# karpathy/minbpe

Measured on AMD Instinct MI355X. Metric: BPE merges/sec, higher is better.
Workload: dtype int32; 1 GPU; regex1g: RegexTokenizer.train, 1 GB synth seed 2, vocab 32000; mode=default, parallelism=single

## Files before the change

### minbpe_amd/_native.py

```python
import ctypes as C
import os
import sys

import numpy as np

_HERE = os.path.dirname(os.path.abspath(__file__))
LIB_PATH = os.environ.get("MINBPE_AMD_LIB", os.path.join(_HERE, "lib", "libbpe_hip.so"))

BPE_OK = 0
BPE_E_HIP = -1
BPE_E_ARG = -2
BPE_E_EMPTY_STATS = -3
BPE_E_STATE = -4
BPE_E_CAP = -5
BPE_E_LIMIT = -6
BPE_E_INTERNAL = -7

PROF_KINDS = ("widen", "pair_count", "argmax", "merge", "table", "encode", "decode")

if not os.path.exists(LIB_PATH):
    raise ImportError(
        f"{LIB_PATH} is missing: build it with `python -m minbpe_amd.build` "
        "(hipcc --offload-arch=gfx950). minbpe_amd has no CPU fallback.")

# ... 387 lines not shown
                return 1

        cb = ALLREDUCE_FN(_cb)
        rc = _lib.bpe_dp_train_cb(self._h, num_merges, rank, nranks, C.cast(cb, C.c_void_p), None, _ptr(pairs),
                                  _ptr(counts), _ptr(lens), C.byref(done))
        d = done.value
        self.last_train = dict(
            pairs=list(map(tuple, pairs[:2 * d].reshape(d, 2).tolist())),
            counts=counts[:d].tolist(), lens=lens[:d].tolist(), iter_ms=None, n_done=d)
        if raised:
            raise raised[0]
        self._check(rc)
        return self.last_train

    def encode_batch(self, pairs, merge_ids, data, offsets=None):
        buf = np.frombuffer(data, dtype=np.uint8) if not isinstance(data, np.ndarray) else data
        off, n_off = self._offsets(offsets)
        n_chunks = n_off if off is not None else 1
        pm = np.ascontiguousarray(pairs, dtype=np.int32).reshape(-1)
        M = len(pm) // 2
        mi = None if merge_ids is None else np.ascontiguousarray(merge_ids, dtype=np.int32)
        out = np.empty(max(len(buf), 1), np.int32)
        oo = np.zeros(n_chunks + 1, np.uint64)
        n_out = _u64(0)
        self._check(_lib.bpe_encode_batch(self._h, _ptr(pm) if M else None, _ptr(mi), M,
                                          _ptr(buf) if len(buf) else None, len(buf), _ptr(off),
                                          n_off, _ptr(out), _ptr(oo), C.byref(n_out)))
        return out[:n_out.value], oo

    def encode_batch_resident(self, pairs, merge_ids, d_bytes: int, n: int, d_offsets: int, n_chunks: int,
                              d_ids_out: int, d_out_offsets: int) -> int:
        p = np.ascontiguousarray(pairs, dtype=np.int32).reshape(-1)
        mids = None if merge_ids is None else np.ascontiguousarray(merge_ids, dtype=np.int32)
        total = _u64(0)
        self._check(_lib.bpe_encode_batch_resident(
            self._h, _ptr(p) if len(p) else None, None if mids is None else _ptr(mids), len(p) // 2,
            C.c_void_p(d_bytes), n, C.c_void_p(d_offsets), n_chunks, C.c_void_p(d_ids_out), C.c_void_p(d_out_offsets),
            C.byref(total)))
        return int(total.value)

    def decode_set_vocab(self, blob: bytes, offsets):
        buf = np.frombuffer(blob, dtype=np.uint8)
        off = np.ascontiguousarray(offsets, dtype=np.uint64)
        self._check(_lib.bpe_decode_set_vocab(self._h, _ptr(buf) if len(buf) else None, _ptr(off),
                                              len(off) - 1))

    def decode_batch(self, ids, doc_offsets=None):
        arr = np.ascontiguousarray(ids, dtype=np.int32)
        nb, bad = _u64(0), _u64(0)
        rc = _lib.bpe_decode_batch(self._h, _ptr(arr) if len(arr) else None, len(arr), C.byref(nb),
                                   C.byref(bad))
        if rc == BPE_E_ARG and bad.value != 0xFFFFFFFFFFFFFFFF:
            raise InvalidToken(int(bad.value))
        self._check(rc)
        out = np.empty(max(nb.value, 1), np.uint8)
        if doc_offsets is None:
            self._check(_lib.bpe_decode_read(self._h, _ptr(out), len(out), None, 0, None))
            return out[:nb.value].tobytes()
        doff = np.ascontiguousarray(doc_offsets, dtype=np.uint64)
        boff = np.zeros(len(doff), np.uint64)
        self._check(_lib.bpe_decode_read(self._h, _ptr(out), len(out), _ptr(doff), len(doff), _ptr(boff)))
        return out[:nb.value].tobytes(), boff

    def decode_set_sparse(self, sparse_ids, v_dense: int):
        arr = np.ascontiguousarray(sparse_ids, dtype=np.int32)
        self._check(_lib.bpe_decode_set_sparse(self._h, _ptr(arr) if len(arr) else None, len(arr), int(v_dense)))

    def decode_batch_resident(self, d_ids: int, id_width: int, n: int, d_doc_off: int, k: int, d_out: int, out_cap: int,
                              d_boff: int) -> int:
        nb, bad = _u64(0), _u64(0)
        rc = _lib.bpe_decode_batch_resident(self._h, C.c_void_p(d_ids), id_width, n, C.c_void_p(d_doc_off), k,
                                            C.c_void_p(d_out), out_cap, C.c_void_p(d_boff), C.byref(nb), C.byref(bad))
        if rc == BPE_E_ARG and bad.value != 0xFFFFFFFFFFFFFFFF:
            raise InvalidToken(int(bad.value))
        if rc == BPE_E_CAP:
            raise OutputTooSmall(int(nb.value), (_lib.bpe_last_error(self._h) or b"").decode())
        self._check(rc)
        return int(nb.value)

    def prof_reset(self):
        self._check(_lib.bpe_prof_reset(self._h))

    def train_stats(self):
        out = np.zeros(12, np.uint64)
        self._check(_lib.bpe_train_stats_ex(self._h, _ptr(out), 12))
        return dict(dense=int(out[0]), sparse=int(out[1]), index_builds=int(out[2]), slots=int(out[3]),
                    lean=int(out[4]), deferred=int(out[5]), chained=int(out[6]), steps=int(out[7]),
                    selections=int(out[8]), slot_ids=int(out[9]), fused_steps=int(out[10]), aa_in_chain=int(out[11]))

    def prof_read(self):
        k = len(PROF_KINDS)
        ms = np.zeros(k, np.float64)
        launches = np.zeros(k, np.uint64)
        nbytes = np.zeros(k, np.uint64)
        self._check(_lib.bpe_prof_read(self._h, _ptr(ms), _ptr(launches), _ptr(nbytes)))
        return {name: dict(ms=float(ms[i]), launches=int(launches[i]), alg_bytes=int(nbytes[i]))
                for i, name in enumerate(PROF_KINDS)}
```

### minbpe_amd/csrc/api/api_basic.hip

```cpp

extern "C" {

const char *bpe_version(void) { return "minbpe_amd libbpe_hip 0.1 (gfx950)"; }

const char *bpe_last_error(bpe_ctx *ctx) { return ctx ? ctx->err.c_str() : g_create_err.c_str(); }

int bpe_create(int device_id, bpe_ctx **out) {
    if (!out) return fail(nullptr, BPE_E_ARG, "out is NULL");
    *out = nullptr;
    int ndev = 0;
    hipError_t e = hipGetDeviceCount(&ndev);
    if (e != hipSuccess || ndev == 0)
        return fail(nullptr, BPE_E_HIP, "no HIP device available: %s",
                    e != hipSuccess ? hipGetErrorString(e) : "device count is 0");
    if (device_id < 0 || device_id >= ndev)
        return fail(nullptr, BPE_E_ARG, "device %d out of range (%d devices)", device_id, ndev);
    bpe_ctx *c = new bpe_ctx();
    c->device = device_id;
    auto bail = [&](const char *what, hipError_t er) {
        int rc = fail(nullptr, BPE_E_HIP, "%s failed: %s", what, hipGetErrorString(er));
        delete c;
        return rc;
    };
    if ((e = hipSetDevice(device_id)) != hipSuccess) return bail("hipSetDevice", e);
// ... 90 lines not shown
    } else if (!strcmp(name, "rep_max")) {
        if (value < 0 || value > 8) return fail(c, BPE_E_ARG, "rep_max must be 0..8");
        c->rep_max = (int)value;
    } else if (!strcmp(name, "rep_min")) {
        if (value < 0 || value > 8) return fail(c, BPE_E_ARG, "rep_min: 0..8");
        c->rep_min = value;
    } else if (!strcmp(name, "lds_delta")) {
        c->lds_delta = value != 0;
    } else if (!strcmp(name, "exp_no_delta")) {
        c->exp_no_delta = value != 0;
    } else if (!strcmp(name, "tie_window")) {
        c->tie_window = value != 0;
    } else if (!strcmp(name, "tie_index")) {
        c->tie_index = value != 0;
    } else if (!strcmp(name, "sparse_ratio")) {
        if (value < 1 || value > 64) return fail(c, BPE_E_ARG, "sparse_ratio must be 1..64");
        c->sparse_ratio = (int)value;
    } else if (!strcmp(name, "lean")) {
        if (value < 0 || value > 2) return fail(c, BPE_E_ARG, "lean must be 0 (never), 1 (auto) or 2 (always)");
        c->lean = (int)value;
    } else if (!strcmp(name, "lean_backoff")) {
        c->lean_backoff = value != 0;
    } else if (!strcmp(name, "lean_count")) {
        if (value < 0) return fail(c, BPE_E_ARG, "lean_count must be >= 0");
        c->lean_count = value;
    } else if (!strcmp(name, "lean_grid")) {
        if (value < 1 || value > 65535) return fail(c, BPE_E_ARG, "lean_grid must be 1..65535");
        c->lean_grid = (int)value;
    } else if (!strcmp(name, "enc_chain")) {
        c->enc_chain = value != 0;
    } else if (!strcmp(name, "enc_cache")) {
        c->enc_cache = value != 0;
    } else if (!strcmp(name, "enc_hash_bits")) {
        if (value < 0 || value > 40) return fail(c, BPE_E_ARG, "enc_hash_bits must be 0..40");
        c->enc_hash_bits = (int)value;
    } else if (!strcmp(name, "dec_copy")) {
        c->dec_copy = value != 0;
    } else if (!strcmp(name, "dec_window")) {
        if (value < 1024 || value > 32768 || value % 16) return fail(c, BPE_E_ARG, "dec_window: 1024..32768 bytes, a multiple of 16");
        c->dec_window = (int)value;
    } else if (!strcmp(name, "dec_tile")) {
        if (value < 256 || value > 16384 || value % 256) return fail(c, BPE_E_ARG, "dec_tile: 256..16384 tokens, a multiple of 256");
        c->dec_tile = (int)value;
    } else if (!strcmp(name, "prof_stride")) {
        if (value < 1 || value > 1024) return fail(c, BPE_E_ARG, "prof_stride must be 1..1024");
        c->prof_stride = (int)value;
    } else if (!strcmp(name, "lean_select")) {
        c->lean_select = value != 0;
    } else if (!strcmp(name, "aa_sparse")) {
        c->aa_sparse = value != 0;
    } else if (!strcmp(name, "dp_force_comm")) {
        c->dp_force_comm = value != 0;
    } else if (!strcmp(name, "dp_kcap")) {
        if (value < 1 || value > DP_KCAP_MAX) return fail(c, BPE_E_ARG, "dp_kcap must be 1..%d", DP_KCAP_MAX);
        c->dp_kcap = (int)value;
    } else if (!strcmp(name, "fuse_load")) {
        c->fuse_load = value != 0;
    } else if (!strcmp(name, "chain_dense")) {
        c->chain_dense = value != 0;
    } else if (!strcmp(name, "chain_prefetch")) {
        c->chain_prefetch = value != 0;
    } else if (!strcmp(name, "count_is_removed")) {
        c->count_is_removed = value != 0;
    } else if (!strcmp(name, "enc_long")) {
        c->enc_long = value != 0;
    } else if (!strcmp(name, "small_slots")) {
        if (value < 0 || value > 2) return fail(c, BPE_E_ARG, "small_slots: 0, 1 or 2");
        c->small_slots = (int)value;
    } else if (!strcmp(name, "chain_kcap")) {
        if (value < 1 || value > CH_KSWEEP) return fail(c, BPE_E_ARG, "chain_kcap must be 1..%d", CH_KSWEEP);
        c->chain_kcap = (int)value;
    } else if (!strcmp(name, "enc_replay")) {
        if (value < 0 || value > 1) return fail(c, BPE_E_ARG, "enc_replay must be 0 or 1");
        c->enc_replay = (int)value;
    } else if (!strcmp(name, "pinned_upload")) {
        if (value < 0 || value > 1) return fail(c, BPE_E_ARG, "pinned_upload must be 0 or 1");
        c->pinned_upload = (int)value;
    } else if (!strcmp(name, "fuse_step")) {
        if (value < 0 || value > 1) return fail(c, BPE_E_ARG, "fuse_step must be 0 or 1");
        c->fuse_step = (int)value;
    } else if (!strcmp(name, "chain_aa")) {
        if (value < 0 || value > 1) return fail(c, BPE_E_ARG, "chain_aa must be 0 or 1");
        c->chain_aa = (int)value;
    } else if (!strcmp(name, "pool_hint")) {
        if (value < 0 || value > 128) return fail(c, BPE_E_ARG, "pool_hint must be 0..128");
        c->pool_hint = (int)value;
    } else if (!strcmp(name, "chain_scan")) {
        if (value < 1 || value > 255) return fail(c, BPE_E_ARG, "chain_scan must be 1..255");
        c->chain_scan = value;
    } else if (!strcmp(name, "chain")) {
        c->chain = value != 0;
    } else if (!strcmp(name, "lean_chain")) {
        c->lean_chain = value != 0;
    } else if (!strcmp(name, "lean_sum")) {
        c->lean_sum = value != 0;
    } else if (!strcmp(name, "lean_scan")) {
        if (value < 1 || value > 1024) return fail(c, BPE_E_ARG, "lean_scan must be 1..1024");
        c->lean_scan = (int)value;
    } else if (!strcmp(name, "repack_acc")) {
        if (value < 0 || value > 10000) return fail(c, BPE_E_ARG, "repack_acc must be 0..10000");
        c->repack_acc = (int)value;
    } else if (!strcmp(name, "depth")) {
        if (value < 0 || value > 64) return fail(c, BPE_E_ARG, "depth must be 0..64");
        c->depth = (int)value;
    } else {
        return fail(c, BPE_E_ARG, "unknown option '%s'", name);
    }
    return BPE_OK;
}

static int check_offsets(bpe_ctx *c, const uint64_t *chunk_offsets, uint64_t n_chunks, uint64_t n) {
    if (!chunk_offsets) return BPE_OK;
    auto scan = [&](uint64_t lo, uint64_t hi) -> uint64_t {
        uint64_t prev = lo ? chunk_offsets[lo - 1] : 0;
        for (uint64_t i = lo; i < hi; i++) {
            const uint64_t o = chunk_offsets[i];
            if (o < prev || o > n) return i;
            prev = o;
        }
        return ~0ull;
    };
    uint64_t bad = ~0ull;
    const unsigned hw = std::max(1u, std::thread::hardware_concurrency());
    const uint64_t T = n_chunks < (1ull << 22) ? 1 : std::max<uint64_t>(1, std::min<uint64_t>(16, hw / 2));
    if (T == 1) {
        bad = scan(0, n_chunks);
    } else {
        std::vector<uint64_t> first(T, ~0ull);
        std::vector<std::thread> pool;
        const uint64_t per = (n_chunks + T - 1) / T;
        for (uint64_t w = 0; w < T; w++)
            pool.emplace_back([&, w] { first[w] = scan(std::min(n_chunks, w * per), std::min(n_chunks, (w + 1) * per)); });
        for (std::thread &t : pool) t.join();
        for (uint64_t w = 0; w < T; w++) bad = std::min(bad, first[w]);
    }
    if (bad != ~0ull)
        return fail(c, BPE_E_ARG, "chunk_offsets[%llu] = %llu: offsets must ascend and stay <= n = %llu",
                    (unsigned long long)bad, (unsigned long long)chunk_offsets[bad], (unsigned long long)n);
    return BPE_OK;
}

static int load_bytes_impl(bpe_ctx *c, const uint8_t *bytes, uint64_t n, const uint64_t *chunk_offsets,
                           uint64_t n_chunks, const uint8_t *wexp) {
    if (!c || (!bytes && n)) return fail(c, BPE_E_ARG, "bytes is NULL");
    TRY(check_offsets(c, chunk_offsets, n_chunks, n));
    if (n >= (1ull << 32)) return fail(c, BPE_E_LIMIT, "stream of %llu bytes exceeds 2^32-1 per GPU",
                                       (unsigned long long)n);
    if (wexp && !chunk_offsets) return fail(c, BPE_E_ARG, "weights need chunk offsets");
    if (wexp) {
        unsigned __int128 stands_for = 0;
        for (uint64_t i = 0; i < n_chunks; i++) {
            if (wexp[i] > 31) return fail(c, BPE_E_ARG, "weight exponent %u of chunk %llu exceeds 31", wexp[i],
                                          (unsigned long long)i);
            const uint64_t b = chunk_offsets[i], e = i + 1 < n_chunks ? chunk_offsets[i + 1] : n;
            if (e > b && e <= n) stands_for += (unsigned __int128)(e - b) << wexp[i];
        }
        if (stands_for >= ((unsigned __int128)1 << 32))
            return fail(c, BPE_E_LIMIT, "the weighted chunks stand for >= 2^32 bytes of text (32-bit pair counts)");
    }
    HIPCHK(c, hipSetDevice(c->device));
    if (n + 16 > c->cap_bytes) {
        TRY(dev_realloc(c, c->d_bytes, (size_t)n + 16));
        c->cap_bytes = n + 16;
    }
    if (n) TRY(upload_h2d(c, c->d_bytes, bytes, n));
    static const uint64_t zero = 0;
// ... 233 lines not shown
```

### minbpe_amd/csrc/api/api_ctx.hip

```cpp

struct DpComm {
    bpe_allreduce_fn fn = nullptr;
    void *user = nullptr;
    int rank = 0, nranks = 1;
};

struct bpe_ctx {
    int device = 0;
    int num_cus = 256;
    hipStream_t stream = nullptr;
    bool own_stream = false;
    std::string err;

    uint8_t *d_bytes = nullptr;
    uint64_t nbytes = 0, cap_bytes = 0;
    uint64_t *d_offsets = nullptr;
    uint64_t n_chunks = 0, cap_offsets = 0;
    bool have_bytes = false;
    uint8_t *d_wexp = nullptr;
    const struct DpComm *dp_comm = nullptr;
    long long *d_dp_ckey = nullptr;
    uint32_t *d_dp_cfold = nullptr;
    uint64_t cap_dp_cfold = 0;
    bool dp_force_comm = false;
// ... 17 lines not shown

    DevState *d_st = nullptr;
    uint64_t *d_tsum = nullptr, *d_tile_off = nullptr;
    uint8_t *d_tile_sin = nullptr;
    unsigned long long *d_sup = nullptr;
    uint64_t cap_tiles = 0;
    IterRec *h_rec = nullptr;
    int rec_cap = 0;
    unsigned long long *d_scratch = nullptr;
    uint32_t *d_delta = nullptr;
    uint32_t *d_dirty_list = nullptr;
    uint32_t *d_dirty_n = nullptr;
    int depth = 8;
    int repack_acc = 200;
    double repack_waste = 0.0;
    int use_slots = 2;
    int fused_rows = 0;
    uint32_t sel_epoch = 0;
    unsigned long long apply_target = 0;
    int rep_shift = 5;
    bool slotted = false;
    uint64_t slot_T = 0;
    int mq = 0;
    uint32_t *d_meta[2] = {nullptr, nullptr};
    uint4 *d_hdr[2] = {nullptr, nullptr};
    uint32_t *d_slot_lens = nullptr;
    unsigned long long *d_slot_off = nullptr, *d_slot_bsum = nullptr;
    uint32_t *d_ids2 = nullptr;
    bool slot2 = false;
    SlotHdr *d_hdr2[2] = {nullptr, nullptr};
    StageRec *d_stage = nullptr;
    uint32_t *d_smask = nullptr;
    uint32_t *d_cand = nullptr;
    uint32_t *d_idx = nullptr;
    uint32_t *d_idx_tmp = nullptr;
    uint32_t *d_idx_dirty = nullptr;
    uint32_t *d_removed = nullptr;
    uint64_t idx_cap_words = 0;
    uint64_t idx_cap_rows = 0;
    bool idx_rebuild = false;
    bool last_aa_indexed = false;
    bool idx_live = false;
    int use_sparse = 1;
    int rep_max = 8;
    int rep_min = 4;
    int lds_delta = 1;
    int exp_no_delta = 0;
    int tie_window = 0;
    int tie_index = 1;
    int sparse_ratio = 1;
    uint64_t last_count = ~0ull;
    uint64_t n_sparse = 0, n_dense = 0, n_index_builds = 0;
    uint64_t n_lean = 0, n_deferred = 0;
    int lean = 1;
    int64_t lean_count = 1 << 20;
    int lean_backoff = 1;
    int lean_grid = 256;
    int lean_scan = 31;
    int lean_select = 1;
    int aa_sparse = 1;
    int lean_chain = 1;
    int chain_dense = 1;
    unsigned long long *d_chain_req = nullptr;
    int ts = TILE2_MAX;
    int small_slots = 1;
    int count_is_removed = 1;
    int chain_prefetch = 1;
    int chain_kcap = CH_KSWEEP;
    int fuse_step = 0;
    unsigned long long *d_step_pub = nullptr;
    uint32_t *d_step_bar = nullptr;
    uint32_t step_bar_target = 0;
    bool forced = false;
    int32_t *d_forced = nullptr;
    uint64_t cap_forced = 0;
    int enc_replay = 1;
    int pinned_upload = 1;
    uint8_t *h_stage = nullptr;
    hipEvent_t ev_stage[4] = {nullptr, nullptr, nullptr, nullptr};
    bool stage_busy[4] = {false, false, false, false};
    uint64_t n_fused = 0;
    int chain_aa = 1;
    uint64_t n_aa_chain = 0;
    unsigned long long *d_step_stamps = nullptr;
    int pool_hint = 0;
    PoolEnt *d_pool = nullptr;
    uint32_t *d_pool_gather = nullptr;
    int chain_scan = 127;
    int chain = 1;
    StepRec *h_srec = nullptr;
    uint64_t n_steps = 0, n_full = 0, n_chained = 0;
    int lean_sum = 1;
    uint4 *d_lean_sum = nullptr;
    bool sum_valid = false;
    uint32_t *d_dbits = nullptr;
    unsigned long long *d_lean_res = nullptr;
    uint32_t lean_tag = 0;
    bool rows_pending = false;
    uint64_t cap_slots = 0;
    int dp_rank = 0, dp_nranks = 1, dp_merges = 0, dp_enq = 0, dp_done = 0;
    bool dp_active = false;
    void *comm = nullptr;
    int comm_rank = 0, comm_nranks = 1;
    uint32_t *d_dp_folded = nullptr, *d_dp_table = nullptr;
    long long *d_dp_key = nullptr;
    uint64_t dp_cur_len = 0;
    bool dp_sparse = false;
    uint32_t dp_dl = 0;
    std::vector<uint8_t> dp_flip;
    int merge_impl = 0;
    unsigned long long *d_desc = nullptr;
    unsigned long long *d_gdesc = nullptr;
    uint64_t cap_desc = 0;
    uint32_t epoch = 0;
    uint32_t lb_tune = 1;

    uint32_t *d_enc_tmp = nullptr, *d_enc_len = nullptr;
    int32_t *d_enc_out = nullptr;
    unsigned long long *d_enc_off = nullptr, *d_enc_bsum = nullptr, *d_enc_long = nullptr;
    unsigned long long *d_enc_huge = nullptr;
    int enc_long = 1;
    unsigned long long *d_ht_keys = nullptr;
    uint32_t *d_ht_vals = nullptr;
    int32_t *d_merge_ids = nullptr;
    uint64_t cap_enc_n = 0, cap_enc_chunks = 0, cap_ht = 0, cap_merge_ids = 0;
    EncEntry *d_enc_tab = nullptr;
    uint32_t *d_enc_rep = nullptr;
    uint8_t *d_enc_mid = nullptr;
    uint32_t *d_enc_midn = nullptr;
    uint64_t cap_enc_tab = 0;
    int enc_cache = 1;
    int enc_chain = 1;
    int enc_hash_bits = 0;

    uint8_t *d_dec_blob = nullptr, *d_dec_out = nullptr;
    unsigned long long *d_dec_voff = nullptr, *d_dec_off = nullptr, *d_dec_bsum = nullptr;
    int32_t *d_dec_ids = nullptr;
    uint32_t *d_dec_len = nullptr;
    uint64_t cap_dec_blob = 0, cap_dec_voff = 0, cap_dec_n = 0, cap_dec_out = 0;
    uint32_t dec_V = 0;
    bool dec_have_vocab = false, dec_have_result = false;
    uint64_t dec_n = 0, dec_total = 0;
    int32_t *d_dec_sparse = nullptr;
    uint64_t cap_dec_sparse = 0;
    uint32_t dec_V_dense = 0, dec_n_sparse = 0;
    int dec_copy = 1;
    int dec_window = 8192;
    int dec_tile = 1024;

    int mode = 1;
    int profile = 0;
    int prof_iter = -1;
    int prof_stride = 64;
    bool prof_active = false;
    int scan_sup_min = 1024;
    int k1 = 2;
    bool stream_is_bytes = false;

    std::vector<ProfEv> prof_open;
    std::vector<hipEvent_t> ev_pool;
    double prof_ms[BPE_PROF_NKINDS] = {0};
    uint64_t prof_launches[BPE_PROF_NKINDS] = {0};
    uint64_t prof_bytes[BPE_PROF_NKINDS] = {0};
};

#define GK(c, kern) ((c)->ts == TILE2_MIN ? bpe::bpe_g1::kern : bpe::bpe_g4::kern)
// ... 812 lines not shown
    const uint32_t T = (uint32_t)c->slot_T;
    const uint32_t dl = delta_layout(c, newid);
    AbArgs A;
    A.b0 = c->d_ids[0];
    A.b1 = c->d_ids[1];
    A.hdr_in = c->d_hdr2[c->mq];
    A.hdr_out = nullptr;
    A.stage = c->d_stage;
    A.smask = c->d_smask;
    A.T = T;
    A.st = c->d_st;
    A.newid = newid;
    A.delta = c->d_delta;
    A.vcap = dl;
    A.idx = c->idx_live ? c->d_idx : nullptr;
    A.istride = (uint32_t)c->idx_cap_words;
    A.cand = nullptr;
    A.removed = c->d_removed;
    A.dirty_n = c->d_dirty_n;
    const uint32_t nwords = (T + 31) / 32;
    const unsigned g = std::max(1u, std::min(use_index ? nwords : (T + 15) / 16, (unsigned)c->lean_grid));
    TRY(prof_begin(c, BPE_PROF_MERGE, 0));
    if (c->idx_live)
        hipLaunchKernelGGL(GK(c, k_merge_ab_lean<true>), dim3(g), dim3(LEAN_MT), 0, c->stream, A, c->d_idx_dirty,
                           use_index ? 1u : 0u, c->d_dbits);
    else
        hipLaunchKernelGGL(GK(c, k_merge_ab_lean<false>), dim3(g), dim3(LEAN_MT), 0, c->stream, A, (const uint32_t *)nullptr, 0u,
                           c->d_dbits);
    LAUNCHCHK(c, "k_merge_ab_lean");
    TRY(prof_end(c));
    TRY(prof_begin(c, BPE_PROF_TABLE, 0));
    const uint32_t na = (newid + 1 + 255) / 256;
    const uint32_t ncommit = std::max(8u, std::min(128u, (nwords + 255) / 256));
    hipLaunchKernelGGL(GK(c, k_apply_lean), dim3(na + ncommit), dim3(256), 0, c->stream, c->d_mat, c->vcap, c->d_delta, dl,
                       c->d_rowmax, c->d_st, newid, c->d_dbits, c->par, rec, iter, na, c->d_hdr2[c->mq], c->d_stage,
                       c->d_removed, c->d_smask, nwords, c->d_lean_sum);
    LAUNCHCHK(c, "k_apply_lean");
    TRY(prof_end(c));
    c->par ^= 1;
    c->stats_valid = false;
    c->stream_is_bytes = false;
    c->rows_pending = true;
    c->n_lean++;
    if (use_index) c->n_sparse++; else c->n_dense++;
    return BPE_OK;
}

int launch_chain_step(bpe_ctx *c, uint32_t step, uint32_t zhi, bool use_index, bool records, bool dense = false) {
    const uint32_t T = (uint32_t)c->slot_T;
    const uint32_t dl = delta_layout(c, zhi);
    const bool fused = c->fuse_step && !c->forced && !dense && !c->dp_comm && use_index && c->idx_live;
    if (!fused) TRY(prof_begin(c, BPE_PROF_ARGMAX, 0));
    CandArgs C;
    C.idx = c->d_idx;
    C.dirty = c->d_idx_dirty;
    C.cand = nullptr;
    C.stride = (uint32_t)c->idx_cap_words;
    C.T = T;
    C.enable = 0;
    C.tie_index = 1;
    C.tie_window = 0;
    C.aa = 0;
    if (!c->idx_live) C.T = 0;
    if (dense && c->dp_comm) C.T = 0;
    (void)records;
    if (!c->d_chain_req) {
        HIPCHK(c, hipMalloc((void **)&c->d_chain_req, PL_REQ_WORDS * sizeof(unsigned long long)));
        HIPCHK(c, hipMemsetAsync(c->d_chain_req, 0, PL_REQ_WORDS * sizeof(unsigned long long), c->stream));
    }
    if (!c->d_pool) {
        HIPCHK(c, hipMalloc((void **)&c->d_pool, (3 * PL_CAP + 128) * sizeof(PoolEnt)));
        HIPCHK(c, hipMalloc((void **)&c->d_pool_gather, (2 + 2 * PL_GATHER) * sizeof(uint32_t)));
        HIPCHK(c, hipMemsetAsync(c->d_pool, 0, (3 * PL_CAP + 128) * sizeof(PoolEnt), c->stream));
        HIPCHK(c, hipMemsetAsync(c->d_pool_gather, 0, (2 + 2 * PL_GATHER) * sizeof(uint32_t), c->stream));
    }
    const DpComm *dp = c->dp_comm;
    uint32_t kcap = (uint32_t)(dense ? CH_KDENSE : std::min(CH_KSWEEP, c->chain_kcap));
    if (dp) kcap = std::min(kcap, (uint32_t)c->dp_kcap);
    if (fused) kcap = std::min(kcap, (uint32_t)STEP_KCAP);
    const uint32_t hint_below = (uint32_t)(c->pool_hint > 0 ? c->pool_hint : (int)kcap);
    const unsigned nscan = (unsigned)std::max(1, std::min(c->chain_scan, c->num_cus - 1));
    const bool aa_on = c->chain_aa && !fused && !c->forced && !dense && !dp && c->lean == 1 && c->idx_live && c->aa_sparse &&
                       c->ts == TILE2_MIN && c->d_desc != nullptr;
    if (fused) {
        if (!c->d_step_pub) {
            HIPCHK(c, hipMalloc((void **)&c->d_step_pub, 64 * sizeof(unsigned long long)));
            HIPCHK(c, hipMemsetAsync(c->d_step_pub, 0, 64 * sizeof(unsigned long long), c->stream));
        }
        if (!c->d_step_bar) {
            HIPCHK(c, hipMalloc((void **)&c->d_step_bar, 256));
            HIPCHK(c, hipMemsetAsync(c->d_step_bar, 0, 256, c->stream));
            c->step_bar_target = 0;
        }
        const uint32_t nwords = (T + 31) / 32;
        StepArgs S;
        S.rowmax = c->d_rowmax;
        S.mat = c->d_mat;
        S.stride = c->vcap;
        S.st = c->d_st;
        S.ref = stream_ref_h(c);
        S.C = C;
        S.dbits = c->d_dbits;
        S.res = c->d_lean_res;
        S.tag = ++c->lean_tag;
        S.req = c->d_chain_req;
        S.kcap = kcap;
        S.pool = c->d_pool;
        S.gather = c->d_pool_gather;
        S.hint_below = hint_below;
        AbArgs &A = S.A;
        A.b0 = c->d_ids[0];
        A.b1 = c->d_ids[1];
        A.hdr_in = c->d_hdr2[c->mq];
        A.hdr_out = nullptr;
        A.stage = c->d_stage;
        A.smask = c->d_smask;
        A.T = T;
        A.st = c->d_st;
        A.newid = 0;
        A.delta = c->d_delta;
        A.vcap = dl;
        A.idx = c->d_idx;
        A.istride = (uint32_t)c->idx_cap_words;
        A.cand = nullptr;
        uint32_t *const removed = (c->weighted || !c->count_is_removed) ? c->d_removed : nullptr;
        A.removed = removed;
        A.dirty_n = c->d_dirty_n;
        S.idx_dirty = c->d_idx_dirty;
        S.use_index = 1u | (c->chain_prefetch ? 2u : 0u);
        const unsigned gapply = (zhi + 1 + 1023) / 1024;
        const unsigned cap = std::min((unsigned)c->num_cus, std::max(std::max((unsigned)c->lean_grid, gapply), 2u));
        const unsigned gmerge = std::max(1u, std::min(std::min(nwords, (unsigned)c->lean_grid), cap));
        const unsigned ns = std::min(nscan, cap - 1);
        const unsigned G = std::min(cap, std::max(std::max(gmerge, gapply), 1 + ns));
        if (G < gapply) return fail(c, BPE_E_INTERNAL, "fused chain step: %u workgroups cannot hold %u tokens", G, zhi + 1);
        S.nscan = ns;
        S.gm = gmerge;
        S.delta = c->d_delta;
        S.dl = dl;
        S.par = c->par;
        S.rec = c->h_rec;
        S.srec = c->h_srec;
        S.step = step;
        S.hdr_cur = c->d_hdr2[c->mq];
        S.stage = c->d_stage;
        S.removed = removed;
        S.smask = c->d_smask;
        S.nwords = nwords;
        S.sums = c->d_lean_sum;
        S.pub = c->d_step_pub;
        S.bar = c->d_step_bar;
        c->step_bar_target += G;
        S.bar_target = c->step_bar_target;
        S.stamps = c->d_step_stamps;
        TRY(prof_begin(c, BPE_PROF_MERGE, 0));
        hipLaunchKernelGGL(GK(c, k_step), dim3(G), dim3(LEAN_MT), 0, c->stream, S);
        LAUNCHCHK(c, "k_step");
        TRY(prof_end(c));
        c->par ^= 1;
        c->stats_valid = false;
        c->stream_is_bytes = false;
        c->rows_pending = true;
        c->n_steps++;
        c->n_fused++;
        c->n_sparse++;
        return BPE_OK;
    }
    if (c->forced)
        hipLaunchKernelGGL(GK(c, k_forced_sel), dim3(1), dim3(64), 0, c->stream, c->d_st, c->d_forced, c->d_mat, c->vcap, kcap);
    else
        hipLaunchKernelGGL(GK(c, k_pool_sel), dim3(1 + nscan), dim3(1024), 0, c->stream, c->d_rowmax, c->d_mat,
                           c->vcap, c->d_st, stream_ref_h(c), C, c->d_dbits, c->d_lean_res, ++c->lean_tag, c->d_chain_req,
                           kcap, c->d_pool, c->d_pool_gather, hint_below, dp ? c->d_dp_ckey : (long long *)nullptr,
                           (unsigned long long)(dp ? dp->rank : 0), c->d_pool + PL_CAP, aa_on ? 1u : 0u);
    LAUNCHCHK(c, "k_pool_sel");
    if (dp) {
        TRY(dp_allreduce(c, c->d_dp_ckey, DP_KEY_WORDS, BPE_DT_INT64, BPE_OP_MIN));
        hipLaunchKernelGGL(GK(c, k_pool_sel_dp), dim3(1), dim3(PL_CAP), 0, c->stream, c->d_st, c->d_dp_ckey, kcap, c->d_pool,
                           c->d_pool + PL_CAP, hint_below);
        LAUNCHCHK(c, "k_pool_sel_dp");
    }
    TRY(prof_end(c));
    AbArgs A;
    A.b0 = c->d_ids[0];
    A.b1 = c->d_ids[1];
    A.hdr_in = c->d_hdr2[c->mq];
    A.hdr_out = dense ? c->d_hdr2[c->mq ^ 1] : nullptr;
    A.stage = c->d_stage;
    A.smask = c->d_smask;
    A.T = T;
    A.st = c->d_st;
    A.newid = 0;
    A.delta = c->d_delta;
    A.vcap = dl;
    A.idx = c->idx_live ? c->d_idx : nullptr;
    A.istride = (uint32_t)c->idx_cap_words;
    A.cand = nullptr;
    uint32_t *const removed = (c->weighted || dp || !c->count_is_removed) ? c->d_removed : nullptr;
    A.removed = removed;
    A.dirty_n = c->d_dirty_n;
    const uint32_t nwords = (T + 31) / 32;
    TRY(prof_begin(c, BPE_PROF_MERGE, 0));
    if (dense) {
        const unsigned g = std::max(1u, std::min((T + 15) / 16, (unsigned)c->num_cus));
        hipLaunchKernelGGL(GK(c, k_merge_chain_dense), dim3(g), dim3(LEAN_MT), 0, c->stream, A, c->d_dbits);
        const unsigned g1 = std::max(1u, std::min((T + MT / 64 - 1) / (MT / 64), 5u * (unsigned)c->num_cus));
        hipLaunchKernelGGL(GK(c, k_merge_chain_dense1), dim3(g1), dim3(MT), 0, c->stream, A);
    } else {
        unsigned g = std::max(1u, std::min(use_index ? nwords : (T + 15) / 16, (unsigned)c->lean_grid));
        ChainAa X;
        X.sdesc = c->d_desc;
        X.removed = c->d_removed;
        X.epoch = 0;
        X.on = aa_on ? 1u : 0u;
        if (aa_on) {
            g = std::min(g, (unsigned)std::max(1, c->num_cus));
            if ((++c->epoch & EPOCH_MASK) == 0) {
                HIPCHK(c, hipMemsetAsync(c->d_desc, 0, ((TILE / TILE2_MIN) * c->cap_tiles + 4) * sizeof(unsigned long long), c->stream));
                c->epoch++;
            }
            X.epoch = c->epoch;
        }
        hipLaunchKernelGGL(GK(c, k_merge_chain), dim3(g), dim3(LEAN_MT), 0, c->stream, A, c->d_idx_dirty,
                           (use_index ? 1u : 0u) | (c->chain_prefetch ? 2u : 0u), c->d_dbits, X);
    }
    LAUNCHCHK(c, "k_merge_chain");
    TRY(prof_end(c));
    TRY(prof_begin(c, BPE_PROF_TABLE, 0));
    const uint32_t na = (zhi + 1 + 255) / 256;
    const uint32_t ncommit = std::max(8u, std::min(128u, (nwords + 255) / 256));
    const uint32_t fS = std::min<uint32_t>(c->vcap, ((zhi + 1 + 63) / 64) * 64);
    uint32_t *ftail = dp ? c->d_dp_cfold + (size_t)2 * kcap * fS : nullptr;
    if (dp) {
        hipLaunchKernelGGL(GK(c, k_dp_fold_chain), dim3(na), dim3(256), 0, c->stream, c->d_delta, dl, c->d_st, c->d_dp_cfold, fS, ftail);
        LAUNCHCHK(c, "k_dp_fold_chain");
        TRY(dp_allreduce(c, c->d_dp_cfold, (uint64_t)2 * kcap * fS + 64, BPE_DT_INT32, BPE_OP_SUM));
    }
    hipLaunchKernelGGL(GK(c, k_apply_chain), dim3(na + ncommit), dim3(256), 0, c->stream, c->d_mat, c->vcap, c->d_delta, dl, c->d_rowmax,
                       c->d_st, c->d_dbits, c->par, c->h_rec, c->h_srec, step, na, c->d_hdr2[c->mq], c->d_stage,
                       removed, c->d_smask, nwords, c->d_lean_sum, dp ? c->d_dp_cfold : (const uint32_t *)nullptr, fS,
                       (const uint32_t *)ftail, aa_on ? c->d_removed : (uint32_t *)nullptr);
    LAUNCHCHK(c, "k_apply_chain");
    TRY(prof_end(c));
    c->par ^= 1;
    if (dense) c->mq ^= 1;
    c->stats_valid = false;
    c->stream_is_bytes = false;
    c->rows_pending = true;
    c->n_steps++;
    if (use_index) c->n_sparse++; else c->n_dense++;
    return BPE_OK;
}

constexpr size_t STAGE_PIECE = 32u << 20;
constexpr int STAGE_R = 4, STAGE_T_MAX = 16;
int upload_h2d(bpe_ctx *c, void *dst, const void *src, size_t bytes) {
    if (!bytes) return BPE_OK;
// ... 121 lines not shown
```

### minbpe_amd/csrc/api/api_prof.hip

```cpp

extern "C" {

int bpe_prof_reset(bpe_ctx *c) {
    if (!c) return BPE_E_ARG;
    TRY(prof_drain(c));
    for (int k = 0; k < BPE_PROF_NKINDS; k++) {
        c->prof_ms[k] = 0;
        c->prof_launches[k] = 0;
        c->prof_bytes[k] = 0;
    }
    return BPE_OK;
}

int bpe_prof_read(bpe_ctx *c, double *ms, uint64_t *launches, uint64_t *alg_bytes) {
    if (!c) return BPE_E_ARG;
    TRY(prof_drain(c));
    for (int k = 0; k < BPE_PROF_NKINDS; k++) {
        if (ms) ms[k] = c->prof_ms[k];
        if (launches) launches[k] = c->prof_launches[k];
        if (alg_bytes) alg_bytes[k] = c->prof_bytes[k];
    }
    return BPE_OK;
}

int bpe_train_stats(bpe_ctx *c, uint64_t *out4) {
    if (!c || !out4) return BPE_E_ARG;
    out4[0] = c->n_dense;
    out4[1] = c->n_sparse;
    out4[2] = c->n_index_builds;
    out4[3] = c->slot_T;
    return BPE_OK;
}

int bpe_train_stats_ex(bpe_ctx *c, uint64_t *out, int n) {
    if (!c || !out || n < 0) return BPE_E_ARG;
    uint64_t chained = 0;
    if (n > 6 && c->d_st) {
        DevState stt;
        TRY(read_state(c, &stt));
        chained = stt.chain_taken;
    }
    const uint64_t v[12] = {c->n_dense, c->n_sparse, c->n_index_builds, c->slot_T, c->n_lean, c->n_deferred,
                            chained + c->n_chained, c->n_steps, c->n_full, (uint64_t)c->ts, c->n_fused, c->n_aa_chain};
    for (int i = 0; i < n && i < 12; i++) out[i] = v[i];
    return BPE_OK;
}

}
```

### minbpe_amd/csrc/api/api_rccl.hip

```cpp

namespace {
struct RcclUid { char internal[128]; };
struct RcclApi {
    void *h = nullptr;
    int (*GetUniqueId)(RcclUid *) = nullptr;
    int (*CommInitRank)(void **, int, RcclUid, int) = nullptr;
    int (*AllReduce)(const void *, void *, size_t, int, int, void *, hipStream_t) = nullptr;
    int (*CommDestroy)(void *) = nullptr;
    int (*CommAbort)(void *) = nullptr;
    const char *(*GetErrorString)(int) = nullptr;
};
constexpr int RCCL_INT32 = 2, RCCL_INT64 = 4, RCCL_SUM = 0, RCCL_MIN = 3;

RcclApi *rccl() {
    static RcclApi api;
    static bool tried = false;
    if (!tried) {
        tried = true;
        for (const char *name : {"librccl.so.1", "librccl.so", "/opt/rocm/lib/librccl.so.1"}) {
            api.h = dlopen(name, RTLD_NOW | RTLD_LOCAL);
            if (api.h) break;
        }
        if (api.h) {
            api.GetUniqueId = (int (*)(RcclUid *))dlsym(api.h, "ncclGetUniqueId");
// ... 15 lines not shown
                        rccl()->GetErrorString ? rccl()->GetErrorString(r_) : "rccl error"); \
    } while (0)
}

extern "C" int bpe_comm_available(void) { return rccl() ? 1 : 0; }

extern "C" int bpe_comm_unique_id(uint8_t *out128) {
    if (!out128) return BPE_E_ARG;
    RcclApi *r = rccl();
    if (!r) return fail(nullptr, BPE_E_HIP, "librccl not found");
    RcclUid id;
    if (r->GetUniqueId(&id) != 0) return fail(nullptr, BPE_E_HIP, "ncclGetUniqueId failed");
    memcpy(out128, id.internal, 128);
    return BPE_OK;
}

extern "C" int bpe_comm_init(bpe_ctx *c, int32_t rank, int32_t nranks, const uint8_t *id128) {
    if (!c || !id128 || rank < 0 || nranks < 1 || rank >= nranks) return fail(c, BPE_E_ARG, "bad arguments");
    RcclApi *r = rccl();
    if (!r) return fail(c, BPE_E_HIP, "librccl not found");
    HIPCHK(c, hipSetDevice(c->device));
    if (c->comm) {
        r->CommDestroy(c->comm);
        c->comm = nullptr;
    }
    RcclUid id;
    memcpy(id.internal, id128, 128);
    RCCLCHK(c, r->CommInitRank(&c->comm, nranks, id, rank));
    c->comm_rank = rank;
    c->comm_nranks = nranks;
    return BPE_OK;
}

extern "C" int bpe_comm_destroy(bpe_ctx *c) {
    if (!c) return BPE_E_ARG;
    if (c->comm && rccl()) {
        (void)hipSetDevice(c->device);
        (void)hipStreamSynchronize(c->stream);
        rccl()->CommDestroy(c->comm);
    }
    c->comm = nullptr;
    return BPE_OK;
}

namespace {
int dp_train_loop(bpe_ctx *c, int32_t num_merges, const DpComm &comm, int32_t *pairs_out, uint64_t *counts_out,
                  uint64_t *len_out, int32_t *n_done) {
    if (n_done) *n_done = 0;
    if (c->mode != 1 || c->use_slots != 2 || c->merge_impl != 0)
        return fail(c, BPE_E_STATE, "sharded training needs the default engine (mode 1, slots 2, merge 0)");
    struct CommScope {
        bpe_ctx *c;
        ~CommScope() { c->dp_comm = nullptr; }
    } scope{c};
    c->dp_comm = &comm;
    TRY(bpe_dp_begin(c, num_merges, comm.rank, comm.nranks));
    TRY(ensure_srec(c));
    if (!c->d_dp_ckey) HIPCHK(c, hipMalloc((void **)&c->d_dp_ckey, DP_KEY_WORDS * sizeof(long long)));
    const uint64_t cfold_words = (uint64_t)2 * DP_KCAP_MAX * c->vcap + 64;
    if (cfold_words > c->cap_dp_cfold) {
        TRY(dev_realloc(c, c->d_dp_cfold, (size_t)cfold_words));
        c->cap_dp_cfold = cfold_words;
    }
    HIPCHK(c, hipMemsetAsync(c->d_dp_cfold, 0, cfold_words * sizeof(uint32_t), c->stream));
    HIPCHK(c, hipMemsetAsync(c->d_dp_ckey, 0, DP_KEY_WORDS * sizeof(long long), c->stream));
    TRY(dp_allreduce(c, c->d_dp_table, 2 * 256 * 256, BPE_DT_INT32, BPE_OP_SUM));
    TRY(bpe_dp_table_ready(c));

    enum { U_GENERAL = 0, U_CHAIN = 2 };
    struct Unit {
        int kind, iter;
        uint32_t step;
        uint8_t hdr_flip, pass_kind;
    };
    std::deque<Unit> q;
    std::vector<long long> lens((size_t)std::max(num_merges, 1), 0);
    int done = 0, rc = BPE_OK, n_chain_inflight = 0;
    uint32_t steps = 0;
    bool stop = false, in_chain = false;
    int general_until = -1, defer_hold = 0, defer_strikes = 0;
    uint64_t lean_at_last_defer = 0, n_chain_merges = 0;
    c->n_lean = c->n_deferred = 0;
    c->n_aa_chain = 0;
    c->n_steps = c->n_full = c->n_chained = 0;
    c->rows_pending = false;
    c->sum_valid = false;

    auto take_record = [&](int j) -> int {
        volatile IterRec *r = &c->h_rec[j];
        if (r->status == ST_EMPTY) {
            stop = true;
            rc = fail(c, BPE_E_EMPTY_STATS, "max() arg is an empty sequence (iteration %d)", j);
            return BPE_OK;
        }
        if (r->status != ST_OK) {
            stop = true;
            rc = fail(c, BPE_E_INTERNAL, "sharded training failed at iteration %d (device status %u)", j, r->status);
            return BPE_OK;
        }
        if (pairs_out) {
            pairs_out[2 * j] = r->a;
            pairs_out[2 * j + 1] = r->b;
        }
        if (counts_out) counts_out[j] = r->count;
        lens[(size_t)j] = (long long)r->new_len;
        if (c->profile) c->prof_bytes[BPE_PROF_MERGE] += 4 * (2 * c->dp_cur_len + r->new_len);
        c->dp_cur_len = r->new_len;
        c->n = r->new_len;
        c->last_count = r->count;
        if (r->a == r->b && c->idx_live && !aa_through_index(c)) c->idx_rebuild = true;
        done = j + 1;
        c->dp_done = done;
        return BPE_OK;
    };
    auto wait_iter = [&](int j) -> int {
        volatile IterRec *r = &c->h_rec[j];
        for (uint64_t spins = 1; r->seq != (unsigned long long)j + 1; spins++) {
            if ((spins & 0xFFFF) == 0 && hipStreamQuery(c->stream) == hipSuccess && r->seq != (unsigned long long)j + 1)
                return fail(c, BPE_E_INTERNAL, "iteration %d never reported (stream idle)", j);
        }
        __sync_synchronize();
        return BPE_OK;
    };
    auto wait_step = [&](uint32_t s) -> int {
        volatile StepRec *r = &c->h_srec[s % STEP_RING];
        for (uint64_t spins = 1; r->seq != (unsigned long long)s + 1; spins++) {
            if ((spins & 0xFFFF) == 0 && hipStreamQuery(c->stream) == hipSuccess && r->seq != (unsigned long long)s + 1)
                return fail(c, BPE_E_INTERNAL, "chain step %u never reported (stream idle)", s);
        }
        __sync_synchronize();
        return BPE_OK;
    };
    auto handle_deferral = [&](bool a_eq_b) -> int {
        HIPCHK(c, hipStreamSynchronize(c->stream));
        for (const Unit &u : q) {
            if (u.kind == U_CHAIN) c->n_steps--;
            if (u.pass_kind == 1) c->n_sparse--; else if (u.pass_kind == 2) c->n_dense--;
        }
        q.clear();
        n_chain_inflight = 0;
        hipLaunchKernelGGL(GK(c, k_clear_defer_chain), dim3(1), dim3(1), 0, c->stream, c->d_st);
        LAUNCHCHK(c, "k_clear_defer_chain");
        c->rows_pending = true;
        c->n_deferred++;
        if (c->lean_backoff && !a_eq_b) {
            defer_strikes = (n_chain_merges - lean_at_last_defer < 16) ? defer_strikes + 1 : 0;
            lean_at_last_defer = n_chain_merges;
            defer_hold = defer_strikes >= 2 ? std::min(32 << std::min(defer_strikes - 2, 5), 1024) : 0;
        } else if (a_eq_b) {
            defer_hold = 0;
        }
        general_until = done + 1 + defer_hold;
        in_chain = false;
        return BPE_OK;
    };

    while (!stop && done < num_merges) {
        const int lb = done + (int)q.size();
        bool enqueued = false;
        if (lb < num_merges && (int)q.size() <= c->depth) {
            const int i = lb;
            const bool want_chain = c->chain && c->lean && c->lean_select && c->tie_index && i > 0 && i >= general_until &&
                                    c->last_count != ~0ull && c->last_count <= (uint64_t)c->lean_count;
            const int hi_dense = std::min(num_merges, done + (int)q.size() * CH_KDENSE + CH_KDENSE);
            const bool want_dense = !want_chain && c->chain && c->chain_dense && c->lean && c->lds_delta && i > 0 &&
                                    i >= general_until && c->last_count != ~0ull && 256 + hi_dense + 1 <= (int)CH_DCAP;
// ... 164 lines not shown
```

### minbpe_amd/csrc/api/api_train.hip

```cpp

extern "C" {

int bpe_train(bpe_ctx *c, int32_t num_merges, int32_t *pairs_out, uint64_t *counts_out,
              double *iter_ms_out, uint64_t *len_out, int32_t *n_done) {
    if (!c || num_merges < 0) return fail(c, BPE_E_ARG, "bad arguments");
    if (!c->have_bytes) return fail(c, BPE_E_STATE, "bpe_load_bytes first");
    if (c->dp_active) return fail(c, BPE_E_STATE, "bpe_dp_end first");
    static const bool timing = getenv("BPE_TIMING") != nullptr;
    auto now = [] { return std::chrono::steady_clock::now(); };
    auto t_begin = now();
    struct ProfIterReset {
        bpe_ctx *c;
        ~ProfIterReset() { c->prof_iter = -1; }
    } prof_iter_reset{c};
    if (n_done) *n_done = 0;
    HIPCHK(c, hipSetDevice(c->device));
    TRY(ensure_table(c, 256u + (uint32_t)num_merges));
    TRY(ensure_rec(c, std::max(num_merges, 1)));
    memset(c->h_rec, 0, sizeof(IterRec) * (size_t)std::max(num_merges, 1));
    TRY(ensure_srec(c));
    const bool delta = (c->mode == 1);
    EventList ev_list;
    std::vector<hipEvent_t> &evs = ev_list.v;
    struct EvSpan {
        int ev, first, k;
    };
    std::vector<EvSpan> ev_spans;
    auto record_event = [&]() -> int {
        hipEvent_t e = nullptr;
        if (hipEventCreate(&e) != hipSuccess) return -1;
        evs.push_back(e);
        if (hipEventRecord(e, c->stream) != hipSuccess) return -1;
        return (int)evs.size() - 1;
    };
    TRY(prof_begin(c, BPE_PROF_TABLE, 0));
    HIPCHK(c, hipMemsetAsync(c->d_mat, 0, (size_t)c->vcap * c->vcap * sizeof(uint32_t), c->stream));
    HIPCHK(c, hipMemsetAsync(c->d_delta, 0, ((size_t)c->vcap * 4 * DELTA_REPL + 256 * DELTA_SKEW) * sizeof(uint32_t), c->stream));
    HIPCHK(c, hipMemsetAsync(c->d_rowmax, 0, (size_t)c->vcap * 2 * sizeof(uint32_t), c->stream));
    HIPCHK(c, hipMemsetAsync(c->d_dbits, 0, DBITS_WORDS * sizeof(uint32_t), c->stream));
    TRY(prof_end(c));
    if (iter_ms_out && record_event() < 0) return fail(c, BPE_E_HIP, "hipEventRecord failed");
    const bool fused_load = load_count_fusable(c);
    TRY(start_from_bytes(c, fused_load));
    const uint64_t n0 = c->n;
    if (!fused_load) TRY(launch_pair_count(c, false));

    int done = 0, rc = BPE_OK;
    uint64_t cur_len = n0;
    bool stop = false;
    c->rep_shift = 5;
    const bool slots = delta && c->use_slots && c->merge_impl == 0;
    const bool form2 = slots && c->use_slots == 2;
    c->idx_live = false;
    c->idx_rebuild = false;
    c->last_count = ~0ull;
    c->n_sparse = c->n_dense = c->n_index_builds = 0;
    c->n_lean = c->n_deferred = 0;
    c->n_steps = c->n_full = c->n_chained = 0;
    c->n_fused = 0;
    c->n_aa_chain = 0;
    static const char *stamp_path = getenv("BPE_STEP_STAMPS");
    const size_t stamp_bytes = (size_t)STEP_STAMP_RING * (3 * 16 + 256 * 2) * sizeof(unsigned long long);
    if (stamp_path) {
        if (!c->d_step_stamps) HIPCHK(c, hipMalloc((void **)&c->d_step_stamps, stamp_bytes));
        HIPCHK(c, hipMemsetAsync(c->d_step_stamps, 0, stamp_bytes, c->stream));
    }
    if (c->d_step_bar) {
        HIPCHK(c, hipMemsetAsync(c->d_step_bar, 0, 256, c->stream));
        c->step_bar_target = 0;
    }
    c->rows_pending = false;
    c->sum_valid = false;
    enum { U_GENERAL = 0, U_LEAN = 1, U_CHAIN = 2 };
    struct Unit {
        int kind;
        int iter;
        uint32_t step;
        uint8_t hdr_flip;
        uint8_t aa_indexed;
        uint8_t pass_kind;
        int ev;
    };
    std::deque<Unit> q;
    int n_chain_inflight = 0;
    uint32_t steps = 0;
    int general_until = -1, defer_hold = 0, defer_strikes = 0;
    uint64_t lean_at_last_defer = 0;
    bool lean_on = false;
    bool in_chain = false;
    bool records_ok = false;
    c->ts = TILE2_MAX;
    if (slots) TRY(form2 ? slots2_enter(c) : slots_enter(c));

    int deferred = -1;
    auto take_record = [&](int j, bool aa_indexed) -> int {
        volatile IterRec *r = &c->h_rec[j];
        if (r->status == ST_DEFER) {
            deferred = j;
            return BPE_OK;
        }
        if (r->status == ST_EMPTY) {
            stop = true;
            rc = fail(c, BPE_E_EMPTY_STATS, "max() arg is an empty sequence (iteration %d)", j);
            return BPE_OK;
        }
        if (r->status != ST_OK) {
            stop = true;
            rc = fail(c, BPE_E_INTERNAL, "device status %u at iteration %d%s", r->status, j,
                      r->status == ST_LOOKBACK ? " (look-back wait timed out; set option merge=0)" : "");
            return BPE_OK;
        }
        if (pairs_out) {
            pairs_out[2 * j] = r->a;
            pairs_out[2 * j + 1] = r->b;
        }
        if (counts_out) counts_out[j] = r->count;
        if (len_out) len_out[j] = r->new_len;
        if (c->profile) {
            if (delta) {
                c->prof_bytes[BPE_PROF_MERGE] += 4 * (2 * cur_len + r->new_len);
            } else {
                c->prof_bytes[BPE_PROF_MERGE] += 4 * (cur_len + r->new_len);
                if (j > 0) c->prof_bytes[BPE_PROF_PAIR_COUNT] += 4 * cur_len;
            }
        }
        cur_len = r->new_len;
        c->n = cur_len;
        c->last_count = r->count;
        if (r->a == r->b && c->idx_live && !aa_indexed) c->idx_rebuild = true;
        c->rep_shift = 5;
        done = j + 1;
        return BPE_OK;
    };
    auto wait_iter = [&](int j) -> int {
        volatile IterRec *r = &c->h_rec[j];
        for (uint64_t spins = 1; r->seq != (unsigned long long)j + 1; spins++) {
            if ((spins & 0xFFFF) == 0 && hipStreamQuery(c->stream) == hipSuccess &&
                r->seq != (unsigned long long)j + 1)
                return fail(c, BPE_E_INTERNAL, "iteration %d never reported (stream idle)", j);
        }
        __sync_synchronize();
        return BPE_OK;
    };
// ... 99 lines not shown
                if (chain) {
                    if (!chain_dense) lean_on = true;
                    if (!in_chain) {
                        TRY(flush_lean_rows(c, c->vcur));
                        hipLaunchKernelGGL(GK(c, k_set_iter), dim3(1), dim3(1), 0, c->stream, c->d_st, (uint32_t)i, (uint32_t)num_merges);
                        LAUNCHCHK(c, "k_set_iter");
                        in_chain = true;
                        records_ok = false;
                    }
                    const int hi = chain_dense ? hi_dense : std::min(num_merges, done + (int)q.size() * CH_KMAX + CH_KMAX);
                    TRY(launch_chain_step(c, steps, 255u + (uint32_t)hi, sparse, records_ok, chain_dense));
                    u.kind = U_CHAIN;
                    u.iter = -1;
                    u.step = steps++;
                    u.pass_kind = sparse ? 1 : 2;
                    u.hdr_flip = chain_dense ? 1 : 0;
                    records_ok = true;
                    n_chain_inflight++;
                    enqueued = true;
                } else if (known) {
                    in_chain = false;
                    records_ok = false;
                    if (lean && !c->forced) {
                        lean_on = true;
                        if (c->lean_select && c->lean_sum && c->sum_valid && c->idx_live && c->tie_index && !full_rowmax) {
                            TRY(launch_sel_lean(c));
                        } else if (c->lean_select && c->idx_live && c->tie_index && !full_rowmax) {
                            TRY(launch_rowsel_lean(c));
                        } else {
                            TRY(flush_lean_rows(c, c->vcur));
                            TRY(launch_select(c, full_rowmax, false));
                        }
                        TRY(launch_lean(c, 256u + (uint32_t)i, i, c->h_rec, sparse));
                        u.kind = U_LEAN;
                        u.pass_kind = sparse ? 1 : 2;
                        c->sum_valid = true;
                    } else {
                        c->sum_valid = false;
                        TRY(flush_lean_rows(c, c->vcur));
                        TRY(launch_select(c, full_rowmax, sparse));
                        if (c->slotted && c->slot2) {
                            const int mq0 = c->mq;
                            TRY(launch_merge2(c, 256u + (uint32_t)i, i, c->h_rec, sparse));
                            u.hdr_flip = (uint8_t)(c->mq != mq0);
                            u.aa_indexed = (uint8_t)c->last_aa_indexed;
                        } else if (c->slotted) {
                            TRY(launch_merge_slot(c, 256u + (uint32_t)i, i, c->h_rec));
                            u.hdr_flip = 1;
                        } else {
                            TRY(launch_merge(c, 256u + (uint32_t)i, i, c->h_rec, delta));
                        }
                    }
                    enqueued = true;
                }
                if (enqueued) {
                    if (iter_ms_out && (u.ev = record_event()) < 0) return fail(c, BPE_E_HIP, "hipEventRecord failed");
                    q.push_back(u);
                }
            }
        }
        if (!q.empty() && ((int)q.size() > c->depth || !enqueued)) {
            const Unit u = q.front();
            if (u.kind == U_CHAIN) {
                TRY(wait_step(u.step));
                const StepRec sr = *const_cast<const StepRec *>(&c->h_srec[u.step % STEP_RING]);
                if (sr.status == ST_DEFER) {
                    if ((int)sr.first_iter != done)
                        return fail(c, BPE_E_INTERNAL, "chain step %u deferred merge %u, the host expected %d", u.step, sr.first_iter, done);
                    TRY(handle_deferral((sr.pad >> 8) == 1));
                } else if (sr.status == ST_EMPTY) {
                    stop = true;
                    rc = fail(c, BPE_E_EMPTY_STATS, "max() arg is an empty sequence (iteration %d)", done);
                } else if (sr.status != ST_OK) {
                    stop = true;
                    rc = fail(c, BPE_E_INTERNAL, "device status %u at iteration %d (chain step %u)", sr.status, done, u.step);
                } else {
                    if (sr.k && (int)sr.first_iter != done)
                        return fail(c, BPE_E_INTERNAL, "chain step %u did merges from %u on, the host expected %d", u.step, sr.first_iter, done);
                    for (uint32_t j = 0; j < sr.k && !stop; j++) {
                        TRY(wait_iter((int)(sr.first_iter + j)));
                        TRY(take_record((int)(sr.first_iter + j), true));
                        if (!stop && c->h_rec[sr.first_iter + j].a == c->h_rec[sr.first_iter + j].b) c->n_aa_chain++;
                    }
                    if (sr.k) {
                        c->n_lean += sr.k;
                        if ((sr.pad & 0xFF) == CH_FULL) c->n_full++;
                        c->n_chained += (sr.pad & 0xFF) == CH_FULL ? sr.k - 1 : sr.k;
                        if (u.ev >= 0) ev_spans.push_back({u.ev, (int)sr.first_iter, (int)sr.k});
                    }
                    q.pop_front();
                    n_chain_inflight--;
                }
            } else {
                TRY(wait_iter(u.iter));
                TRY(take_record(u.iter, u.aa_indexed != 0));
                if (deferred >= 0) {
                    TRY(handle_deferral(c->h_rec[u.iter].a == c->h_rec[u.iter].b));
                } else if (!stop) {
                    if (u.ev >= 0) ev_spans.push_back({u.ev, u.iter, 1});
                    q.pop_front();
                }
            }
        }
        if (done >= num_merges) break;
    }
    c->prof_iter = -1;
    auto t_drain = now();
    HIPCHK(c, hipStreamSynchronize(c->stream));
    if (!stop) {
        for (const Unit &u : q) {
            if (u.kind == U_CHAIN) c->n_steps--;
            if (u.pass_kind == 1) c->n_sparse--; else if (u.pass_kind == 2) c->n_dense--;
        }
        q.clear();
        TRY(flush_lean_rows(c, 256u + (uint32_t)done));
    }
    c->rows_pending = false;
    auto t_tail = now();
    if (c->slotted) {
        if (stop) {
            const int back = (int)q.size();
            if (back & 1) c->par ^= 1;
            if (c->slot2) {
                for (const Unit &u : q)
                    if (u.hdr_flip) c->mq ^= 1;
            } else if (back & 1) {
                c->mq ^= 1;
            }
            hipLaunchKernelGGL(k_set_status, dim3(1), dim3(1), 0, c->stream, c->d_st, 0u);
        }
        TRY(c->slot2 ? slots2_leave(c) : slots_leave(c));
        HIPCHK(c, hipStreamSynchronize(c->stream));
        c->n = cur_len;
        c->vcur = 256u + (uint32_t)done;
    } else {
        c->par = done & 1;
        c->n = cur_len;
        c->vcur = 256u + (uint32_t)done;
    }
    if (iter_ms_out) {
        int prev = 0;
        for (const EvSpan &sp : ev_spans) {
            float ms = 0.f;
            HIPCHK(c, hipEventElapsedTime(&ms, evs[(size_t)prev], evs[(size_t)sp.ev]));
            for (int j = 0; j < sp.k; j++)
                if (sp.first + j < done) iter_ms_out[sp.first + j] = ms / sp.k;
            prev = sp.ev;
        }
    }
    TRY(prof_drain(c));
    if (stamp_path && c->d_step_stamps) {
        std::vector<unsigned long long> h(stamp_bytes / sizeof(unsigned long long));
        HIPCHK(c, hipMemcpy(h.data(), c->d_step_stamps, stamp_bytes, hipMemcpyDeviceToHost));
        if (FILE *f = fopen(stamp_path, "wb")) {
            fwrite(h.data(), 1, stamp_bytes, f);
            fclose(f);
        }
    }
    if (timing) {
        auto ms = [](auto a, auto b) { return std::chrono::duration<double, std::milli>(b - a).count(); };
        fprintf(stderr, "[bpe_train] %d merges: setup+enqueue of the first pass %.2f ms, loop %.2f ms, drain %.2f ms, "
                        "re-pack + timers %.2f ms\n", done, ms(t_begin, t_loop), ms(t_loop, t_drain), ms(t_drain, t_tail),
                ms(t_tail, now()));
    }
    if (n_done) *n_done = done;
    return rc;
// ... 4 lines not shown
```

### minbpe_amd/csrc/kernels/k_chain.hip

```cpp
#include <hip/hip_runtime.h>
#include <stdint.h>

#include "../bpe_device.h"

namespace bpe {
namespace BPE_G {

constexpr uint32_t CH_EX_CAP = 2048;

__device__ __forceinline__ int chain_match(const uint32_t *pa, const uint32_t *pb, uint32_t K, uint32_t w0, uint32_t w1) {
    const uint32_t x = w0 & IDMASK, y = w1 & NWMASK;
    int hit = -1;
    for (uint32_t p = 0; p < K; p++)
        if (x == pa[p] && y == pb[p]) hit = (int)p;
    return (w0 == INVALID_WORD) ? -1 : hit;
}

constexpr uint32_t CH_DCAP = 1024;
constexpr uint32_t CH_SD = 2 * CH_DCAP + 2;
__device__ __forceinline__ void chain_slot_load(const AbArgs &A, const uint32_t t, uint4 (&rv)[MJ], uint4 &hv) {
    const int lane = lane_id();
    const uint32_t *src = A.b0 + (size_t)t * TILE2;
#pragma unroll
    for (int j = 0; j < MJ; j++) rv[j] = *reinterpret_cast<const uint4 *>(src + j * 256 + lane * 4);
    hv = (lane & 1) ? make_uint4(INVALID_WORD, INVALID_WORD, 0u, 0u) : make_uint4(INVALID_WORD, INVALID_WORD, INVALID_WORD, 0u);
    const long long hi = 2ll * (long long)t - 2 + lane;
    if (lane < 6 && hi >= 0 && hi < 2ll * (long long)A.T) hv = reinterpret_cast<const uint4 *>(A.hdr_in)[hi];
}
template <bool DENSE, bool THROUGH = false>
__device__ __forceinline__ void merge_chain_wave(uint32_t *__restrict__ out, uint32_t *__restrict__ sd, const uint32_t t, const AbArgs &A,
                                                 const uint32_t *pa, const uint32_t *pb, const uint32_t *pb1,
                                                 const uint32_t K, const uint32_t z0, const uint32_t brep,
                                                 uint4 (&rv)[MJ], const uint4 hv,
                                                 const uint32_t *ph = nullptr, const uint32_t hm = 0,
                                                 const uint32_t tl_in = 0xFFFFFFFFu) {
    const int lane = lane_id();
    const uint32_t Tl = tl_in != 0xFFFFFFFFu ? tl_in : min(A.T, A.st->tlive);
    const uint32_t *src;
    const uint32_t meta = bcast(hv.w, 2);
    const uint32_t len = meta & 0x7FFFFFFFu, buf = meta >> 31;
    auto keep_header = [&]() {
        if (DENSE && (lane == 2 || lane == 3)) reinterpret_cast<uint4 *>(A.hdr_out)[2 * (size_t)t + (lane - 2)] = hv;
    };
    if (len == 0) {
        keep_header();
        return;
    }
    if (buf) {
        src = A.b1 + (size_t)t * TILE2;
#pragma unroll
        for (int j = 0; j < MJ; j++) rv[j] = *reinterpret_cast<const uint4 *>(src + j * 256 + lane * 4);
    }
    const uint32_t first = bcast(hv.x, 2);
    uint32_t halo0 = bcast(hv.x, 4), halo1 = bcast(hv.y, 4), halo2 = bcast(hv.z, 4);
    uint32_t prev2 = bcast(hv.x, 1), prev1 = bcast(hv.y, 1);
    uint32_t tprev = t - 1;
    uint32_t tnext = t + 1;
    {
        const uint32_t nlen = bcast(hv.w, 4) & 0x7FFFFFFFu, plen = bcast(hv.w, 0) & 0x7FFFFFFFu;
        if ((t + 1 < Tl && nlen < 3) || (t > 0 && plen < 2)) {
            uint32_t ctx[7] = {0, 0, 0, 0, 0, 0, 0};
            if (lane == 0) slot_context_walk(A.hdr_in, t, Tl, ctx);
            halo0 = bcast(ctx[0], 0);
            halo1 = bcast(ctx[1], 0);
            halo2 = bcast(ctx[2], 0);
            prev2 = bcast(ctx[3], 0);
            prev1 = bcast(ctx[4], 0);
            tprev = bcast(ctx[5], 0);
            tnext = bcast(ctx[6], 0);
        }
    }
    auto at = [&](int q, uint32_t own) -> uint32_t {
        const int d = q - (int)len;
        return d < 0 ? own : (d == 0 ? halo0 : (d == 1 ? halo1 : (d == 2 ? halo2 : INVALID_WORD)));
    };
    uint32_t x[MJ][4];
#pragma unroll
    for (int j = 0; j < MJ; j++) {
        const int q0 = j * 256 + lane * 4;
        if ((j + 1) * 256 <= (int)len) {
            x[j][0] = rv[j].x;
            x[j][1] = rv[j].y;
            x[j][2] = rv[j].z;
            x[j][3] = rv[j].w;
        } else {
            x[j][0] = at(q0 + 0, rv[j].x);
            x[j][1] = at(q0 + 1, rv[j].y);
            x[j][2] = at(q0 + 2, rv[j].z);
            x[j][3] = at(q0 + 3, rv[j].w);
        }
    }
    uint32_t tail[3];
#pragma unroll
    for (int i = 0; i < 3; i++) tail[i] = at(TILE2 + i, 0u);
    uint32_t rb[MJ], jc[MJ], valid[MJ];
#pragma unroll
    for (int j = 0; j < MJ; j++) {
        rb[j] = 0;
        jc[j] = 0;
    }
    uint32_t s = 0;
    uint32_t ia[MJ];
#pragma unroll
    for (int j = 0; j < MJ; j++) ia[j] = 0;
    uint32_t ip = 0;
    if (hm) {
        auto code = [&](uint32_t w) -> uint32_t {
            const uint32_t id = w & IDMASK;
            const uint32_t e = ph[(__umul24(id, hm) >> 8) & 255u];
            return (e >> 8) == id ? (e & 255u) : 0u;
        };
#pragma unroll
        for (int j = 0; j < MJ; j++) {
#pragma unroll
            for (int k = 0; k < 4; k++) ia[j] |= code(x[j][k]) << (8 * k);
        }
        ip = code(prev1);
    } else {
        for (uint32_t p = 0; p < K; p++) {
            const uint32_t a = pa[p];
#pragma unroll
            for (int j = 0; j < MJ; j++) {
#pragma unroll
                for (int k = 0; k < 4; k++) ia[j] |= ((x[j][k] & IDMASK) == a) ? (p + 1u) << (8 * k) : 0u;
            }
            ip = ((prev1 & IDMASK) == a) ? p + 1u : ip;
        }
    }
#pragma unroll
    for (int j = 0; j < MJ; j++) {
        const uint32_t up = (j < MJ - 1) ? lane_first(x[(j + 1) % MJ][0]) : tail[0];
        const uint32_t nxw = lane_next(x[j][0], up);
#pragma unroll
        for (int k = 0; k < 4; k++) {
            const uint32_t nxt = (k < 3) ? x[j][k + 1] : nxw;
            const uint32_t i = (ia[j] >> (8 * k)) & 255u;
            const uint32_t m = (uint32_t)((nxt & NWMASK) == pb1[i]);
            rb[j] |= m << k;
            jc[j] |= (m ? i : 0u) << (8 * k);
        }
    }
    s = (uint32_t)((prev1 != INVALID_WORD) & ((first & NWMASK) == pb1[ip]));
#pragma unroll
    for (int j = 0; j < MJ; j++) {
        const int nb = (int)len - (j * 256 + lane * 4);
        valid[j] = nb >= 4 ? 0xFu : (nb <= 0 ? 0u : ((1u << nb) - 1u));
    }
    uint32_t anyr = 0;
#pragma unroll
    for (int j = 0; j < MJ; j++) anyr |= rb[j] & valid[j];
    const bool sites = __any(anyr != 0) != 0;
    if (!sites && !s) {
        keep_header();
        return;
    }
    uint32_t mb[MJ], kb[MJ], ex[MJ], cnt[MJ];
#pragma unroll
    for (int j = 0; j < MJ; j++) {
        mb[j] = rb[j] & valid[j];
        const uint32_t upr = (j > 0) ? ((lane_last(rb[(j + MJ - 1) % MJ]) >> 3) & 1u) : s;
        const uint32_t mp = (uint32_t)dpp_mov<0x138>((int)upr, (int)((rb[j] >> 3) & 1u));
        kb[j] = ~((mb[j] << 1) | mp) & valid[j] & 0xFu;
        cnt[j] = (uint32_t)__popc(kb[j]);
    }
    uint32_t total = 0;
    if constexpr (MJ == 4) {
        const uint32_t i01 = wave_iscan_add(cnt[0] | (cnt[1] << 16));
        const uint32_t i23 = wave_iscan_add(cnt[2] | (cnt[3] << 16));
        const uint32_t t01 = lane_last(i01), t23 = lane_last(i23);
        const uint32_t tot0 = t01 & 0xFFFFu, tot1 = t01 >> 16, tot2 = t23 & 0xFFFFu, tot3 = t23 >> 16;
        ex[0] = (i01 & 0xFFFFu) - cnt[0];
        ex[1] = tot0 + (i01 >> 16) - cnt[1];
        ex[2] = tot0 + tot1 + (i23 & 0xFFFFu) - cnt[2];
        ex[3] = tot0 + tot1 + tot2 + (i23 >> 16) - cnt[3];
        total = tot0 + tot1 + tot2 + tot3;
    } else {
#pragma unroll
        for (int j = 0; j < MJ; j++) {
            const uint32_t inc = wave_iscan_add(cnt[j]);
            ex[j] = total + inc - cnt[j];
            total += lane_last(inc);
        }
    }
    uint32_t fstore = 0;
    if (!s) {
        uint32_t fc = 0x7FFFFFFFu;
#pragma unroll
        for (int j = 0; j < MJ; j++) {
            if (mb[j]) {
                const uint32_t k0 = (uint32_t)__ffs((int)mb[j]) - 1u;
                fc = min(fc, ex[j] + (uint32_t)__popc(kb[j] & ((1u << k0) - 1u)));
            }
        }
        fstore = (uint32_t)wave_min_i32((int)fc) & ~3u;
    }
#pragma unroll
    for (int j = 0; j < MJ; j++) {
        uint32_t o = ex[j];
#pragma unroll
        for (int k = 0; k < 4; k++) {
            if ((kb[j] >> k) & 1u) {
                const uint32_t w = x[j][k];
                const uint32_t z = z0 + ((jc[j] >> (8 * k)) & 255u) - 1u;
                out[o++] = ((mb[j] >> k) & 1u) ? (z | (w & (FLAG | WMASK))) : w;
            }
        }
    }
    __builtin_amdgcn_fence(__ATOMIC_RELEASE, "wavefront");
    __builtin_amdgcn_wave_barrier();
    __builtin_amdgcn_fence(__ATOMIC_ACQUIRE, "wavefront");
    {
        uint32_t *dst = (buf ? A.b1 : A.b0) + (size_t)t * TILE2;
        for (uint32_t i = fstore + (uint32_t)lane * 4; i < total; i += 256)
            *reinterpret_cast<uint4 *>(dst + i) = *reinterpret_cast<const uint4 *>(&out[i]);
    }
    if (lane == 0) {
        uint32_t h[8];
        h[0] = total > 0 ? out[0] : INVALID_WORD;
        h[1] = total > 1 ? out[1] : INVALID_WORD;
        h[2] = total > 2 ? out[2] : INVALID_WORD;
        h[3] = total | (buf << 31);
        h[4] = total > 1 ? out[total - 2] : INVALID_WORD;
        h[5] = total > 0 ? out[total - 1] : INVALID_WORD;
        h[6] = h[7] = 0;
        if (DENSE) {
// ... 153 lines not shown
                if (mu & 0x7FFFFFFFu) break;
            }
            const int lu = (int)(mu & 0x7FFFFFFFu);
            const uint32_t *pu = ((mu >> 31) ? A.b1 : A.b0) + (size_t)u * TILE2;
            int ones = 0;
            bool open = true;
            uint32_t nextw = first;
            for (int base = lu - 1; base >= 0 && open; base -= 64) {
                const int q = base - lane;
                const uint32_t xq = (q >= 0) ? pu[q] : INVALID_WORD;
                uint32_t nx = (uint32_t)__shfl_up((int)xq, 1);
                if (lane == 0) nx = nextw;
                const bool r = (q >= 0) && ((xq & IDMASK) == a) && ((nx & NWMASK) == a);
                const unsigned long long zeros = __ballot(!r);
                if (zeros) {
                    ones += __ffsll((long long)zeros) - 1;
                    const int zl = __ffsll((long long)zeros) - 1;
                    open = (base - zl < 0);
                    break;
                }
                ones += 64;
                nextw = (uint32_t)__shfl((int)xq, 63);
            }
            if (!open || ones < lu) {
                sc = (uint32_t)(ones & 1);
            } else {
                uint32_t su = 0;
                bool got = false;
                for (uint32_t spins = 0; spins < LOOKBACK_SPINS; spins++) {
                    const unsigned long long d = desc_load(&X.sdesc[u]);
                    if ((d >> 42) == (tag >> 42) + (1ull << 20)) {
                        su = (uint32_t)(d & 1u);
                        got = true;
                        break;
                    }
                    __builtin_amdgcn_s_sleep(8);
                }
                failed = !got;
                sc = (uint32_t)(((lu - 1) & 1) == 0) ^ su;
            }
        }
        if (lane == 0) {
            desc_store(&X.sdesc[t], tag | (1ull << 62) | sc);
            if (failed) atomicExch(&A.st->status, ST_LOOKBACK);
        }
        s = sc;
    }
    {
        uint32_t anyr = s;
        const int q0 = lane * 4;
        const int nb = len + 1 - q0;
        const uint32_t keep = nb >= 4 ? 0xFu : (nb <= 0 ? 0u : ((1u << nb) - 1u));
        anyr |= tl.rb[0] & keep;
        if (len == TILE2) anyr |= (uint32_t)(((tl.tail[0] & IDMASK) == a) & ((tl.tail[1] & NWMASK) == a));
        if (!__any(anyr != 0)) return;
    }
    tile_lzscan<true>(tl, nullptr);
    uint32_t kept = 0;
    bool changed = false;
    uint32_t *dst = (cur ? A.b0 : A.b1) + (size_t)t * TILE2;
    tile_rewrite<true, true, 1, true>(tl, s, a, a, newid, dst, nullptr, A.delta, A.vcap, len, &kept, &changed, s_hdr, A.idx,
                                      A.istride, t, tnext, t);
    __builtin_amdgcn_fence(__ATOMIC_RELEASE, "wavefront");
    __builtin_amdgcn_wave_barrier();
    __builtin_amdgcn_fence(__ATOMIC_ACQUIRE, "wavefront");
    if (lane == 0 && changed) {
        uint32_t h[8];
        h[0] = kept > 0 ? s_hdr[0] : INVALID_WORD;
        h[1] = kept > 1 ? s_hdr[1] : INVALID_WORD;
        h[2] = kept > 2 ? s_hdr[2] : INVALID_WORD;
        h[3] = kept | ((cur ^ 1u) << 31);
        h[4] = kept > 1 ? s_hdr[4] : INVALID_WORD;
        h[5] = kept > 0 ? s_hdr[5] : INVALID_WORD;
        h[6] = h[7] = 0;
        stage_put<false>(A.stage + t, t, h);
        atomicOr(&A.smask[t >> 5], 1u << (t & 31));
        atomicAdd(&X.removed[(t & 255u) * REMOVED_STRIDE], (uint32_t)len - kept);
        if (kept < 3 && t + 1 < Tl) A.st->gap = 1;
    }
    __builtin_amdgcn_fence(__ATOMIC_RELEASE, "wavefront");
    __builtin_amdgcn_wave_barrier();
}

__device__ __forceinline__ uint32_t chain_hash_find(const uint32_t *pa, uint32_t K, uint32_t *tab) {
    if (K < 5) return 0u;
    const uint32_t lane = (uint32_t)lane_id(), half = lane >> 5, l = lane & 31u;
    const bool in = l < K;
    const uint32_t a = in ? pa[l] : 0u;
    volatile uint32_t *t = tab + half * 256u;
    for (uint32_t m = 129u; m < 256u; m += 4u) {
        const uint32_t h = (__umul24(a, m + 2u * half) >> 8) & 255u;
        if (in) t[h] = l;
        __builtin_amdgcn_fence(__ATOMIC_RELEASE, "wavefront");
        __builtin_amdgcn_wave_barrier();
        __builtin_amdgcn_fence(__ATOMIC_ACQUIRE, "wavefront");
        const bool clash = in && t[h] != l;
        const unsigned long long cb = __ballot(clash);
        if ((uint32_t)cb == 0u) return m;
        if ((uint32_t)(cb >> 32) == 0u) return m + 2u;
    }
    return 0u;
}
__device__ __forceinline__ uint32_t chain_hash_build(uint32_t *s_ph, uint32_t *s_hm, uint32_t *s_hs, const uint32_t *s_pa, uint32_t K,
                                                     bool pre_ok = false, uint32_t pre_hm = 0) {
    if (threadIdx.x < 256) s_ph[threadIdx.x] = 0xFFFFFFFFu;
    uint32_t hm = pre_hm;
    if (!pre_ok) {
        if (threadIdx.x == 0) *s_hm = 0;
        __syncthreads();
        if (wave_id() == 0) {
            const uint32_t f = chain_hash_find(s_pa, K, s_hs);
            if (lane_id() == 0) *s_hm = f;
        }
        __syncthreads();
        hm = *s_hm;
    } else {
        __syncthreads();
    }
    if (hm && threadIdx.x < K) s_ph[(__umul24(s_pa[threadIdx.x], hm) >> 8) & 255u] = (s_pa[threadIdx.x] << 8) | (threadIdx.x + 1u);
    __syncthreads();
    return hm;
}

struct MergeLds {
    alignas(16) uint32_t s_out[LEAN_MT / 64][TILE2];
    uint32_t s_list[LEAN_SUB * 32];
    uint32_t s_tot[2];
    uint32_t s_pa[CH_KMAX], s_pb[CH_KMAX], s_pb1[CH_KMAX + 1];
    uint32_t s_ph[256], s_hm;
    uint32_t s_hs[512];
};
template <bool THROUGH = false>
__device__ __forceinline__ void merge_chain_body(const AbArgs &A, const uint32_t *__restrict__ idx_dirty, uint32_t use_index,
                                                 MergeLds &L, const uint32_t K, const uint32_t z0, const uint32_t brep,
                                                 const uint32_t blk, const uint32_t nblk, unsigned long long *dbg = nullptr,
                                                 const bool have_st = false, const uint32_t tlive_in = 0, const uint32_t gap_in = 0,
                                                 const bool pre_ok = false, const uint32_t pre_hm = 0, const ChainAa *X = nullptr) {
    auto dstamp = [&](int i) {
        if (dbg && threadIdx.x == 0) dbg[i] = wall_clock64();
    };
    DevState *st = A.st;
    auto &s_out = L.s_out;
    auto &s_list = L.s_list;
    auto &s_tot = L.s_tot;
    auto &s_pa = L.s_pa;
    auto &s_pb = L.s_pb;
    auto &s_pb1 = L.s_pb1;
    const uint32_t hm = chain_hash_build(L.s_ph, &L.s_hm, L.s_hs, s_pa, K, pre_ok, pre_hm);
    const uint32_t *s_ph = L.s_ph;
    const uint32_t Tl = min(A.T, have_st ? tlive_in : st->tlive);
    const uint32_t gap = have_st ? gap_in : st->gap;
    constexpr uint32_t NWV = LEAN_MT / 64;
    AbArgs A1 = A;
    A1.newid = z0;
    const uint32_t a0 = s_pa[0], b0 = s_pb[0];
    const bool aa = MJ == 1 && X != nullptr && X->on && K == 1 && a0 == b0;
    auto do_slot = [&](uint32_t t) {
        if constexpr (MJ == 1) {
            if (aa) {
                merge_aa_wave(s_out[wave_id()], t, A, *X, a0, z0, Tl);
                return;
            }
        }
        if (K == 1) {
            merge_ab_wave<true, true, false, THROUGH>(s_out[wave_id()], nullptr, t, A1, a0, b0, Tl);
        } else {
            uint4 rv[MJ], hv;
            chain_slot_load(A, t, rv, hv);
            merge_chain_wave<false, THROUGH>(s_out[wave_id()], nullptr, t, A, s_pa, s_pb, s_pb1, K, z0, brep, rv, hv, s_ph, hm, Tl);
        }
    };
    if (!(use_index & 1u) || gap != 0) {
        const uint32_t nw = nblk * NWV;
        for (uint32_t t = blk * NWV + wave_id(); t < Tl; t += nw) do_slot(t);
        return;
    }
    dstamp(8);
    const uint32_t nwords = (Tl + 31) / 32;
    const uint32_t per = (nwords + nblk - 1) / nblk;
    const uint32_t wlo = blk * per, whi = min(nwords, wlo + per);
    for (uint32_t sub = wlo; sub < whi; sub += LEAN_SUB) {
        uint32_t mk = 0;
        const uint32_t w = sub + threadIdx.x;
        if (threadIdx.x < LEAN_SUB && w < whi) {
            mk = idx_dirty[w];
            for (uint32_t p = 0; p < K; p++) {
                uint32_t h1, h2, h3;
                pair_hash(s_pa[p], s_pb[p], h1, h2, h3);
                mk |= A.idx[(size_t)h1 * A.istride + w] & A.idx[(size_t)h2 * A.istride + w] &
                      A.idx[(size_t)h3 * A.istride + w];
            }
            if (aa) {
                uint32_t nx = 0;
                if (w + 1 < nwords) {
                    uint32_t h1, h2, h3;
                    pair_hash(a0, a0, h1, h2, h3);
                    nx = idx_dirty[w + 1] | (A.idx[(size_t)h1 * A.istride + w + 1] & A.idx[(size_t)h2 * A.istride + w + 1] &
                                             A.idx[(size_t)h3 * A.istride + w + 1]);
                }
                mk |= (mk >> 1) | (nx << 31);
            }
            const uint32_t left = Tl - w * 32;
            if (left < 32) mk &= (1u << left) - 1u;
        }
        const uint32_t c = (uint32_t)__popc(mk);
        const uint32_t inc = wave_iscan_add(c);
        if (threadIdx.x < 128 && lane_id() == 63) s_tot[wave_id()] = inc;
        __syncthreads();
        const uint32_t n = s_tot[0] + s_tot[1];
        if (threadIdx.x < LEAN_SUB) {
            uint32_t o = inc - c + (wave_id() == 1 ? s_tot[0] : 0u);
            while (mk) {
                s_list[o++] = w * 32 + (uint32_t)__ffs((int)mk) - 1u;
                mk &= mk - 1u;
            }
        }
        __syncthreads();
        if (sub == wlo) dstamp(9);
        if (K == 1 || MJ > 1 || !(use_index & 2u)) {
            for (uint32_t i = wave_id(); i < n; i += NWV) do_slot(s_list[i]);
        } else {
            uint32_t i = wave_id();
            uint4 rv[MJ], hv, nrv[MJ], nhv;
            if (i < n) chain_slot_load(A, s_list[i], rv, hv);
            for (; i < n; i += NWV) {
                const bool more = i + NWV < n;
                if (more) chain_slot_load(A, s_list[i + NWV], nrv, nhv);
                merge_chain_wave<false, THROUGH>(s_out[wave_id()], nullptr, s_list[i], A, s_pa, s_pb, s_pb1, K, z0, brep, rv, hv, s_ph, hm, Tl);
                if (more) {
#pragma unroll
                    for (int j = 0; j < MJ; j++) rv[j] = nrv[j];
                    hv = nhv;
                }
            }
        }
        __syncthreads();
    }
}
enum { SW_BB = CH_KMAX, SW_BADJ = 2 * CH_KMAX, SW_BK = 3 * CH_KMAX, SW_BZ0, SW_BREP, SW_STATUS, SW_DEFER, SW_SEL_RAN, SW_TLIVE, SW_GAP, SW_BHM, SW_BHM_KEY, SW_ADJ, SW_N };
constexpr int SW_WORDS = 128;
static_assert(SW_N <= SW_WORDS, "two waves fetch the state words");
__device__ __forceinline__ void step_words_fetch(const DevState *st, uint32_t *s_w) {
    const uint32_t i = threadIdx.x;
    if (i < (uint32_t)SW_N) {
        const uint32_t *base = reinterpret_cast<const uint32_t *>(st);
        uint32_t off;
        if (i < (uint32_t)SW_BB) off = (uint32_t)offsetof(DevState, ba) / 4 + i;
        else if (i < (uint32_t)SW_BADJ) off = (uint32_t)offsetof(DevState, bb) / 4 + (i - (uint32_t)SW_BB);
        else if (i < (uint32_t)SW_BK) off = (uint32_t)offsetof(DevState, badj) / 4 + (i - (uint32_t)SW_BADJ);
        else {
            constexpr uint32_t o[SW_N - SW_BK] = {
                (uint32_t)offsetof(DevState, bk) / 4,      (uint32_t)offsetof(DevState, bz0) / 4,     (uint32_t)offsetof(DevState, brep) / 4,
                (uint32_t)offsetof(DevState, status) / 4,  (uint32_t)offsetof(DevState, defer) / 4,   (uint32_t)offsetof(DevState, sel_ran) / 4,
                (uint32_t)offsetof(DevState, tlive) / 4,   (uint32_t)offsetof(DevState, gap) / 4,     (uint32_t)offsetof(DevState, bhm) / 4,
                (uint32_t)offsetof(DevState, bhm_key) / 4, (uint32_t)offsetof(DevState, adj) / 4};
            off = o[0];
#pragma unroll
            for (int k = 1; k < SW_N - SW_BK; k++) off = (i == (uint32_t)SW_BK + (uint32_t)k) ? o[k] : off;
        }
        s_w[i] = base[off];
    }
    __syncthreads();
}
__global__ void __launch_bounds__(LEAN_MT)
k_merge_chain(AbArgs A, const uint32_t *__restrict__ idx_dirty, uint32_t use_index, uint32_t *__restrict__ dbits, ChainAa X) {
    __shared__ MergeLds L;
    __shared__ uint32_t s_w[SW_WORDS];
    DevState *st = A.st;
    step_words_fetch(st, s_w);
    const uint32_t ran = s_w[SW_SEL_RAN];
    if (blockIdx.x == 0 && ran) {
        for (uint32_t i = threadIdx.x; i < DBITS_WORDS; i += LEAN_MT) dbits[i] = 0;
        __syncthreads();
        if (threadIdx.x == 0) st->sel_ran = 0;
    }
    const uint32_t K = s_w[SW_BK];
    if (s_w[SW_STATUS] || s_w[SW_DEFER] || K == 0) return;
    const uint32_t z0 = s_w[SW_BZ0], brep = s_w[SW_BREP];
    if (threadIdx.x < CH_KMAX) {
        L.s_pa[threadIdx.x] = threadIdx.x < K ? s_w[threadIdx.x] : 0xFFFFFFFFu;
        L.s_pb[threadIdx.x] = threadIdx.x < K ? s_w[SW_BB + threadIdx.x] : 0xFFFFFFFFu;
        L.s_pb1[threadIdx.x + 1] = threadIdx.x < K ? s_w[SW_BB + threadIdx.x] : 0xFFFFFFFFu;
        if (threadIdx.x == 0) L.s_pb1[0] = 0xFFFFFFFFu;
    }
    __syncthreads();
    if (K == 1 && s_w[0] == s_w[SW_BB] && !(MJ == 1 && X.on)) {
        if (blockIdx.x == 0 && threadIdx.x == 0) atomicExch(&st->status, ST_INTERNAL);
        return;
    }
    merge_chain_body(A, idx_dirty, use_index, L, K, z0, brep, blockIdx.x, gridDim.x, nullptr, true, s_w[SW_TLIVE], s_w[SW_GAP],
                     s_w[SW_BHM_KEY] == ((z0 << 8) | K), s_w[SW_BHM], &X);
}

constexpr int CH_KDENSE = 6;
static_assert((LEAN_MT / 64) * TILE2 * 4 + CH_KDENSE * (int)CH_SD * 4 + 256 <= 160 * 1024, "dense chain pass: LDS");
__global__ void __launch_bounds__(LEAN_MT)
k_merge_chain_dense(AbArgs A, uint32_t *__restrict__ dbits) {
    __shared__ __attribute__((aligned(16))) uint32_t s_out[LEAN_MT / 64][TILE2];
    __shared__ uint32_t s_sd[CH_KDENSE * CH_SD];
    __shared__ uint32_t s_pa[CH_KMAX], s_pb[CH_KMAX], s_pb1[CH_KMAX + 1];
    DevState *st = A.st;
    const uint32_t ran = st->sel_ran;
    if (blockIdx.x == 0 && ran) {
        for (uint32_t i = threadIdx.x; i < DBITS_WORDS; i += LEAN_MT) dbits[i] = 0;
        __syncthreads();
        if (threadIdx.x == 0) st->sel_ran = 0;
    }
    const uint32_t K = st->bk;
    if (!(st->status || st->defer) && K == 1) return;
    if (st->status || st->defer || K == 0 || K > (uint32_t)CH_KDENSE) {
        const uint4 *hi = reinterpret_cast<const uint4 *>(A.hdr_in);
        uint4 *ho = reinterpret_cast<uint4 *>(A.hdr_out);
        for (size_t i = (size_t)blockIdx.x * LEAN_MT + threadIdx.x; i < 2 * (size_t)A.T; i += (size_t)gridDim.x * LEAN_MT) ho[i] = hi[i];
        if (K > (uint32_t)CH_KDENSE && blockIdx.x == 0 && threadIdx.x == 0) st->status = ST_INTERNAL;
        return;
    }
    const uint32_t z0 = st->bz0, brep = st->brep;
    if (threadIdx.x < CH_KMAX) {
        s_pa[threadIdx.x] = threadIdx.x < K ? (uint32_t)st->ba[threadIdx.x] : 0xFFFFFFFFu;
        s_pb[threadIdx.x] = threadIdx.x < K ? (uint32_t)st->bb[threadIdx.x] : 0xFFFFFFFFu;
        s_pb1[threadIdx.x + 1] = threadIdx.x < K ? (uint32_t)st->bb[threadIdx.x] : 0xFFFFFFFFu;
        if (threadIdx.x == 0) s_pb1[0] = 0xFFFFFFFFu;
    }
    for (uint32_t i = threadIdx.x; i < K * CH_SD; i += LEAN_MT) s_sd[i] = 0;
    __syncthreads();
    constexpr uint32_t NWV = LEAN_MT / 64;
    const uint32_t nw = gridDim.x * NWV;
    const uint32_t Tl = min(A.T, st->tlive);
    for (uint32_t t = blockIdx.x * NWV + wave_id(); t < A.T; t += nw)
    {
        uint4 rv[MJ], hv;
        chain_slot_load(A, t, rv, hv);
        merge_chain_wave<true>(s_out[wave_id()], s_sd, t, A, s_pa, s_pb, s_pb1, K, z0, (uint32_t)CH_RSTRIDE, rv, hv, nullptr, 0, Tl);
    }
    __syncthreads();
    const uint32_t vc = A.vcap & 0xFFFFFFu;
    const uint32_t lim = min(vc, (uint32_t)CH_DCAP);
    for (uint32_t p = 0; p < K; p++) {
        const uint32_t *sd = s_sd + p * CH_SD;
        uint32_t *g = A.delta + delta_rep_off(p * (uint32_t)CH_RSTRIDE + (blockIdx.x & (brep - 1u)), vc);
        for (uint32_t i = threadIdx.x; i < lim; i += LEAN_MT) {
            const uint32_t l = sd[i], r = sd[CH_DCAP + i];
            if (l) atomicAdd(&g[i], l);
            if (r) atomicAdd(&g[vc + i], r);
        }
        if (threadIdx.x == 0) {
            const uint32_t adj = sd[2 * CH_DCAP], rem = sd[2 * CH_DCAP + 1];
            if (adj) atomicAdd(&st->badj[p], adj);
            if (rem && A.removed) atomicAdd(&A.removed[(p * (uint32_t)CH_RMV + (blockIdx.x & (uint32_t)(CH_RMV - 1))) * REMOVED_STRIDE], rem);
        }
    }
}
__global__ void __launch_bounds__(MT, 5)
k_merge_chain_dense1(AbArgs A) {
    __shared__ __attribute__((aligned(16))) uint32_t s_out[MT / 64][TILE2];
    __shared__ uint32_t s_delta[2 * LDSD_CAP + 2];
    const DevState *st = A.st;
    if (st->status || st->defer || st->bk != 1) return;
    const uint32_t a = (uint32_t)st->ba[0], b = (uint32_t)st->bb[0];
    A.newid = st->bz0;
    ldsd_clear(s_delta);
    const uint32_t nw = gridDim.x * (MT / 64);
    const uint32_t Tl = min(A.T, st->tlive);
    for (uint32_t t = blockIdx.x * (MT / 64) + wave_id(); t < A.T; t += nw)
        merge_ab_wave<false, false, true>(s_out[wave_id()], s_delta, t, A, a, b, Tl);
    ldsd_flush(s_delta, A);
}

template <bool OWNED>
__device__ __forceinline__ void apply_chain_tokens(const uint32_t t, uint32_t *__restrict__ mat, uint32_t stride,
                                                   uint32_t *__restrict__ delta, uint32_t vcap, const uint32_t *__restrict__ rowmax,
                                                   uint32_t *__restrict__ dbits, uint4 *__restrict__ sums,
                                                   const uint32_t *__restrict__ folded, uint32_t fS, const uint32_t *__restrict__ ftail,
                                                   const uint32_t K, const uint32_t z0, const uint32_t ran,
                                                   const uint32_t *pairs, const uint32_t *adjs, const uint32_t brep_in) {
    auto dld = [&](const uint32_t *p) -> uint32_t { return OWNED ? ld_agent(p) : *p; };
    auto pair_a = [&](uint32_t p) -> uint32_t { return pairs[p] >> 16; };
    auto pair_b = [&](uint32_t p) -> uint32_t { return pairs[p] & 0xFFFFu; };
    {
        const uint32_t Zlast = z0 + K - 1u;
        if ((t & ~255u) > Zlast) return;
        const bool live = t <= Zlast;
        const uint32_t nrep = 1u << (vcap >> 24);
        const uint32_t vc = vcap & 0xFFFFFFu;
        uint2 rm = make_uint2(0u, 0u);
        uint32_t prevflag = 0, oldword = 0;
        if (OWNED) {
            oldword = ran ? 0u : dbits[t >> 5];
            prevflag = (oldword >> (t & 31)) & 1u;
            if (live) {
                const unsigned long long v = ld_agent64(reinterpret_cast<const unsigned long long *>(rowmax) + t);
                rm = make_uint2((uint32_t)v, (uint32_t)(v >> 32));
            }
        } else if (live) {
            prevflag = (dbits[t >> 5] >> (t & 31)) & 1u;
            rm = reinterpret_cast<const uint2 *>(rowmax)[t];
        }
        bool flagged = false;
        if (!OWNED && K == 1 && pair_a(0) == pair_b(0)) {
            const uint32_t a = pair_a(0), Z = z0;
            constexpr int RB = 4;
            uint32_t acc[4] = {0, 0, 0, 0};
            const uint32_t old_ta = live ? mat[(size_t)t * stride + a] : 0u;
            for (uint32_t r0 = 0; r0 < nrep; r0 += RB) {
                uint32_t x[RB][4];
#pragma unroll
                for (int k = 0; k < RB; k++)
#pragma unroll
                    for (int v = 0; v < 4; v++)
                        x[k][v] = (live && r0 + k < nrep) ? delta[delta_rep_off(r0 + k, vc) + (size_t)v * vc + t] : 0u;
#pragma unroll
                for (int k = 0; k < RB; k++)
#pragma unroll
                    for (int v = 0; v < 4; v++) {
                        if (x[k][v]) delta[delta_rep_off(r0 + k, vc) + (size_t)v * vc + t] = 0;
                        acc[v] += x[k][v];
// ... 251 lines not shown
    const bool noop = status || st->defer || K == 0;
    const uint32_t t = blockIdx.x * 256u + threadIdx.x;
    if (t < 32) tail[t] = t == 16 ? (status ? 1u : 0u) : ((!noop && t < K && t < 16) ? (K == 1 ? st->adj : st->badj[t]) : 0u);
#ifdef BPE_DP_DEBUG
    if (t >= 32 && t < 64) {
        uint32_t v = 0;
        if (t == 32) v = st->iter;
        else if (t == 33) v = st->sel_mode;
        else if (t == 34) v = K;
        else if (t == 35) v = st->tl_n;
        else if (t == 36) v = st->tl_M;
        else if (t == 37) v = st->tl_skip;
        else if (t == 38) v = st->defer;
        else if (t == 39) v = st->gap;
        else if (t < 48) v = (uint32_t)st->ba[t - 40] << 16 | (uint32_t)st->bb[t - 40];
        else v = (uint32_t)st->chain[2 * (t - 48)] << 16 | (uint32_t)st->chain[2 * (t - 48) + 1];
        tail[t] = v;
    }
#endif
    if (noop || t > z0 + K - 1u || t >= S) return;
    const uint32_t nrep = 1u << (dl >> 24), vc = dl & 0xFFFFFFu;
    if (K == 1) {
        uint32_t sl = 0, sr = 0;
        for (uint32_t r = 0; r < nrep; r++) {
            const size_t o = delta_rep_off(r, vc);
            const uint32_t x = delta[o + t], y = delta[o + vc + t];
            if (x) delta[o + t] = 0;
            if (y) delta[o + vc + t] = 0;
            sl += x;
            sr += y;
        }
        folded[t] = sl;
        folded[(size_t)S + t] = sr;
        return;
    }
    const uint32_t brep = st->brep;
    for (uint32_t p = 0; p < K; p++) {
        uint32_t x[CH_RSTRIDE][2];
#pragma unroll
        for (int r = 0; r < CH_RSTRIDE; r++) {
            const size_t o = delta_rep_off(p * (uint32_t)CH_RSTRIDE + (uint32_t)r, vc);
            x[r][0] = (uint32_t)r < brep ? delta[o + t] : 0u;
            x[r][1] = (uint32_t)r < brep ? delta[o + vc + t] : 0u;
        }
        uint32_t sl = 0, sr = 0;
#pragma unroll
        for (int r = 0; r < CH_RSTRIDE; r++) {
            const size_t o = delta_rep_off(p * (uint32_t)CH_RSTRIDE + (uint32_t)r, vc);
            if (x[r][0]) delta[o + t] = 0;
            if (x[r][1]) delta[o + vc + t] = 0;
            sl += x[r][0];
            sr += x[r][1];
        }
        folded[(size_t)(2 * p) * S + t] = sl;
        folded[(size_t)(2 * p + 1) * S + t] = sr;
    }
}
__global__ void k_dp_after_sum(DevState *st, const uint32_t *__restrict__ tail) {
    if (tail[8] != 0 && st->status == 0) st->status = ST_INTERNAL;
}

__global__ void __launch_bounds__(64)
k_forced_sel(DevState *st, const int32_t *__restrict__ pairs, const uint32_t *__restrict__ mat, uint32_t stride, uint32_t kcap) {
    const uint32_t lane = threadIdx.x;
    const uint32_t status = st->status, defer = st->defer, iter = st->iter, nm = st->num_merges;
    if (status || defer) return;
    if (iter >= nm) {
        if (lane == 0) st->bk = 0;
        return;
    }
    const uint32_t r = iter + lane;
    const bool in = lane < kcap && r < nm;
    const uint32_t a = in ? (uint32_t)pairs[2 * r] : 0xFFFFFFFEu, b = in ? (uint32_t)pairs[2 * r + 1] : 0xFFFFFFFDu;
    uint32_t bad = in ? ((a == b) | (a >= 256u + iter) | (b >= 256u + iter)) : 1u;
#pragma unroll
    for (int j = 0; j < CH_KSWEEP - 1; j++) {
        const uint32_t aj = (uint32_t)__shfl((int)a, j), bj = (uint32_t)__shfl((int)b, j);
        if ((uint32_t)j < lane) bad |= (aj == a) | (aj == b) | (bj == a) | (bj == b);
    }
    const unsigned long long bb = __ballot(bad != 0);
    const uint32_t K = bb ? min(kcap, (uint32_t)__ffsll((long long)bb) - 1u) : kcap;
    const uint32_t c = lane < K ? mat[(size_t)a * stride + b] : 0u;
    const uint32_t cmax = wave_umax_dpp(c);
    __shared__ uint32_t s_pa[CH_KMAX], s_hs[512];
    if (lane < CH_KMAX) s_pa[lane] = a;
    __syncthreads();
    const uint32_t hm = chain_hash_find(s_pa, K, s_hs);
    if (lane == 0) {
        st_agent(&st->adj, 0u);
        st->count = c;
        st->ntied = 1;
        st->firstpos = NOPOS;
        st->sel_tie = 0;
        st->a = (int32_t)a;
        st->b = (int32_t)b;
        st->fin_a = (int32_t)a;
        st->fin_b = (int32_t)b;
        st->bk = K;
        st->bz0 = 256u + iter;
        st->tl_n = st->tl_skip = 0;
        st->dp_wait = 0;
        st->sel_mode = CH_LIST;
        st->found = K ? 1u : 0u;
        if (K == 0) st->defer = 1;
        st->brep = cmax > CH_REP_COUNT ? (uint32_t)CH_RSTRIDE : (uint32_t)CH_REP;
        st->bhm = hm;
        st->bhm_key = ((256u + iter) << 8) | K;
        st->pool_n = 0;
    }
    if (lane < K) {
        st->ba[lane] = (int32_t)a;
        st->bb[lane] = (int32_t)b;
        st_agent(&st->badj[lane], 0u);
        st->bcnt[lane] = c;
    }
}
__global__ void k_forced_pair(DevState *st, const int32_t *__restrict__ pairs, uint32_t iter, const uint32_t *__restrict__ mat,
                              uint32_t stride) {
    if (threadIdx.x != 0 || blockIdx.x != 0) return;
    st->adj = 0;
    st->chain_n = 0;
    if (st->status) return;
    const int32_t a = pairs[2 * iter], b = pairs[2 * iter + 1];
    st->a = a;
    st->b = b;
    st->fin_a = a;
    st->fin_b = b;
    st->count = mat[(size_t)(uint32_t)a * stride + (uint32_t)b];
    st->ntied = 1;
    st->firstpos = NOPOS;
    st->sel_tie = 0;
    st->found = 1;
    st->ncand = 0;
}

__global__ void k_set_iter(DevState *st, uint32_t iter, uint32_t num_merges) {
    st->iter = iter;
    st->num_merges = num_merges;
    st->sel_mode = CH_FULL;
    st->tl_n = st->tl_skip = 0;
    st->bk = 0;
    st->scan_a = st->scan_b = st->scan_z = NOROW;
    st->chain_n = 0;
    st->dp_wait = 0;
    st->pool_n = 0;
    st->pool_hint = st->pool_hint_next = 1;
    st->pool_epoch = 0;
}
__global__ void k_clear_defer_chain(DevState *st) {
    st->defer = 0;
    st->chain_n = 0;
    st->sel_mode = CH_FULL;
    st->tl_n = st->tl_skip = 0;
    st->bk = 0;
    st->dp_wait = 0;
    st->pool_n = 0;
    st->pool_hint = st->pool_hint_next = 1;
}

}
}
```

### minbpe_amd/csrc/kernels/k_pool.hip

```cpp
#include <hip/hip_runtime.h>
#include <stdint.h>

#include "../bpe_device.h"

namespace bpe {
namespace BPE_G {

constexpr uint32_t PL_CAP = 256;
constexpr uint32_t PL_ROWS = 128;
constexpr uint32_t PL_GATHER = 1024;
static_assert(PL_GATHER >= 4 * PL_CAP, "maintain: four variants per entry");
constexpr uint32_t PL_REQ_WORDS = 2 + PL_ROWS + 256;

struct PoolScratch {
    uint32_t dl[PL_CAP];
    uint32_t rank[PL_GATHER];
    uint32_t w[8];
    uint32_t wtot[PL_CAP / 64];
    uint32_t fv, nl, k;
    uint32_t bad;
};
__device__ __forceinline__ void pool_sort(const uint32_t *ixy, const uint32_t *ic, const unsigned long long *ikey,
                                          uint32_t *oxy, uint32_t *oc, unsigned long long *okey, uint32_t n, PoolScratch &X) {
    const uint32_t tid = threadIdx.x;
    uint32_t sh = 0;
    while (sh < 4 && (n << (sh + 1)) <= blockDim.x) sh++;
    const uint32_t tpe = 1u << sh, e = tid >> sh, q = tid & (tpe - 1u);
    if (tid < n) X.rank[tid] = 0;
    __syncthreads();
    if (e < n) {
        const uint32_t c = ic[e], x = ixy[e];
        uint32_t r = 0;
#pragma unroll 4
        for (uint32_t j = q; j < n; j += tpe) {
            const uint32_t cj = ic[j];
            r += (cj > c) | ((cj == c) & (ixy[j] < x));
        }
        if (r) atomicAdd(&X.rank[e], r);
    }
    __syncthreads();
    if (tid < n) {
        const uint32_t r = X.rank[tid];
        oxy[r] = ixy[tid];
        oc[r] = ic[tid];
        okey[r] = ikey[tid];
    }
    __syncthreads();
}
constexpr int PL_KSH = 40, PL_KSH_DP = 43, PL_POS_DP = 33;
__device__ __forceinline__ void pool_level_bounds(const uint32_t *c, uint32_t n, uint32_t *ls, uint32_t *le, PoolScratch &X) {
    const uint32_t tid = threadIdx.x, w = (uint32_t)wave_id(), lane = (uint32_t)lane_id();
    const bool in = tid < n;
    const bool start = in && (tid == 0 || c[tid - 1] != c[tid]);
    const unsigned long long bal = __ballot(start);
    if (tid < PL_CAP && lane == 0) {
        X.w[w] = bal ? w * 64u + 63u - (uint32_t)__clzll((long long)bal) : 0xFFFFFFFFu;
        X.w[4 + w] = bal ? w * 64u + (uint32_t)__ffsll((long long)bal) - 1u : 0xFFFFFFFFu;
    }
    __syncthreads();
    if (in) {
        const unsigned long long upto = lane == 63 ? ~0ull : ((2ull << lane) - 1ull);
        const unsigned long long below = bal & upto, above = bal & ~upto;
        uint32_t lo = 0, hi = n;
        if (below) {
            lo = w * 64u + 63u - (uint32_t)__clzll((long long)below);
        } else {
            for (int v = (int)w - 1; v >= 0; v--)
                if (X.w[v] != 0xFFFFFFFFu) {
                    lo = X.w[v];
                    break;
                }
        }
        if (above) {
            hi = w * 64u + (uint32_t)__ffsll((long long)above) - 1u;
        } else {
            for (uint32_t v = w + 1; v < PL_CAP / 64; v++)
                if (X.w[4 + v] != 0xFFFFFFFFu) {
                    hi = X.w[4 + v];
                    break;
                }
        }
        ls[tid] = lo;
        le[tid] = hi;
    }
    __syncthreads();
}
__device__ __forceinline__ void pool_levels_dirty(const unsigned long long *key, uint32_t n, const uint32_t *ls, const uint32_t *le,
                                                  uint32_t *dirty, int ksh, PoolScratch &X) {
    const uint32_t tid = threadIdx.x;
    if (tid < n) X.dl[tid] = 0;
    __syncthreads();
    if (tid < n) {
        const uint32_t lo = ls[tid], hi = le[tid];
        const unsigned long long e0 = key[lo] >> ksh;
        if (hi - lo > 1 && (e0 == 0 || (key[tid] >> ksh) != e0)) X.dl[lo] = 1;
    }
    __syncthreads();
    if (tid < n) dirty[tid] = X.dl[ls[tid]];
    __syncthreads();
}
__device__ __forceinline__ void pool_finish(DevState *st, PoolEnt *__restrict__ pool, const uint32_t *b_xy, const uint32_t *b_c,
                                            const unsigned long long *b_key, uint32_t *a_xy, uint32_t *a_c,
                                            unsigned long long *a_key, const uint32_t *s_ls, const uint32_t *s_le,
                                            uint32_t *s_dirty, uint32_t *s_clash, uint32_t *s_k, uint32_t *s_unt, uint32_t n,
                                            uint32_t kmax, uint32_t iter, uint32_t theta, unsigned long long epoch, bool rebuilt,
                                            uint32_t hint_below, int ksh, PoolScratch &X, const bool aa_ok = false) {
    const uint32_t tid = threadIdx.x;
    const uint32_t nwalk = min(n, kmax);
    const uint32_t sh = blockDim.x >= 4 * PL_CAP ? 2u : 0u;
    const uint32_t tpe = 1u << sh, e = tid >> sh, q = tid & (tpe - 1u);
    if (tid < n) {
        X.rank[tid] = 0;
        X.dl[tid] = 0;
    }
    if (tid == 0) {
        *s_unt = 0;
        X.bad = 0;
    }
    __syncthreads();
    if (e < n) {
        const uint32_t lo = s_ls[e], hi = s_le[e];
        const unsigned long long k = b_key[e];
        uint32_t r = 0;
#pragma unroll 4
        for (uint32_t j = lo + q; j < hi; j += tpe) {
            const unsigned long long kj = b_key[j];
            r += (kj < k) | ((kj == k) & (j < e));
        }
        if (r) atomicAdd(&X.rank[e], r);
        if (q == 0) {
            const unsigned long long e0 = b_key[lo] >> ksh;
            if (hi - lo > 1 && (e0 == 0 || (k >> ksh) != e0)) X.dl[lo] = 1;
        }
    }
    __syncthreads();
    if (tid < n) {
        const uint32_t lo = s_ls[tid];
        const uint32_t r = lo + X.rank[tid];
        a_xy[r] = b_xy[tid];
        a_c[r] = b_c[tid];
        a_key[r] = b_key[tid];
        s_dirty[r] = X.dl[lo];
    }
    __syncthreads();
    for (uint32_t q2 = tid; q2 < 32u * nwalk; q2 += blockDim.x) {
        const uint32_t i = q2 >> 5, j = q2 & 31u;
        const uint32_t x = a_xy[i] >> 16, y = a_xy[i] & 0xFFFFu;
        bool bad = false;
        if (j == i) {
            bad = ((x == y) & !(aa_ok && i == 0)) | (s_dirty[i] != 0);
        } else if (j < i) {
            const uint32_t xj = a_xy[j] >> 16, yj = a_xy[j] & 0xFFFFu;
            if (j == 0 && xj == yj) bad = true;
            bad |= (xj == x) | (xj == y) | (yj == x);
        }
        if (bad) atomicOr(&X.bad, 1u << i);
    }
    __syncthreads();
    if (tid == 0) *s_k = X.bad ? min(nwalk, (uint32_t)__ffs((int)X.bad) - 1u) : nwalk;
    __syncthreads();
    const uint32_t K = *s_k;
    if (tid == 0) {
        st_agent(&st->adj, 0u);
        st->count = a_c[0];
        st->ntied = s_le[0];
        st->firstpos = NOPOS;
        st->sel_tie = 0;
        st->a = (int32_t)(a_xy[0] >> 16);
        st->b = (int32_t)(a_xy[0] & 0xFFFFu);
        st->fin_a = (int32_t)(a_xy[0] >> 16);
        st->fin_b = (int32_t)(a_xy[0] & 0xFFFFu);
        st->bk = K;
        st->bz0 = 256u + iter;
        st->tl_n = st->tl_skip = 0;
        st->dp_wait = 0;
        st->sel_mode = rebuilt ? CH_FULL : CH_LIST;
        if (K == 0) {
            st->found = 0;
            st->defer = ((a_xy[0] >> 16) == (a_xy[0] & 0xFFFFu) && !s_dirty[0]) ? 1u : 2u;
            st->pool_n = 0;
            st->pool_hint_next = 1;
        } else {
            st->found = 1;
        }
    }
    if (K == 0) return;
    if (tid < K) X.rank[tid] = a_xy[tid] >> 16;
    __syncthreads();
    if (tid < 64) {
        uint32_t c = 0;
        if (tid < K) {
            c = a_c[tid];
            st->ba[tid] = (int32_t)(a_xy[tid] >> 16);
            st->bb[tid] = (int32_t)(a_xy[tid] & 0xFFFFu);
            st_agent(&st->badj[tid], 0u);
            st->bcnt[tid] = c;
        }
        const uint32_t cmax = wave_umax_dpp(c);
        const uint32_t hm = chain_hash_find(reinterpret_cast<const uint32_t *>(X.rank), K, X.rank + 256);
        if (tid == 0) {
            st->brep = cmax > CH_REP_COUNT ? (uint32_t)CH_RSTRIDE : (uint32_t)CH_REP;
            st->bhm = hm;
            st->bhm_key = ((256u + iter) << 8) | K;
        }
    }
    const uint32_t Kout = (K == 1 && (a_xy[0] >> 16) == (a_xy[0] & 0xFFFFu)) ? 0u : K;
    bool unt = false;
    if (tid >= Kout && tid < n) {
        PoolEnt e2;
        e2.xy = a_xy[tid];
        e2.c = a_c[tid];
        e2.key = a_key[tid];
        pool[tid - Kout] = e2;
        const uint32_t x = e2.xy >> 16, y = e2.xy & 0xFFFFu;
        bool touched = false;
#pragma unroll 4
        for (uint32_t p = 0; p < K; p++) touched |= ((a_xy[p] & 0xFFFFu) == x) | ((a_xy[p] >> 16) == y);
        unt = !touched;
    }
    if (tid < PL_CAP) {
        const unsigned long long ub = __ballot(unt);
        if (lane_id() == 0 && ub) atomicAdd(s_unt, (uint32_t)__popcll(ub));
    }
    __syncthreads();
    if (tid == 0) {
        st->pool_n = n - Kout;
        st->pool_theta = theta;
        st->pool_epoch = epoch;
        st->pool_hint_next = *s_unt < hint_below ? 1u : 0u;
    }
}

struct PoolLds {
    unsigned long long s_red[32];
    uint32_t s_words[DBITS_WORDS], s_pref[DBITS_WORDS + 1];
    uint32_t s_exrow[CH_EX_CAP], s_exm[CH_EX_CAP], s_exarg[CH_EX_CAP];
    uint32_t a_xy[PL_GATHER], a_c[PL_GATHER], b_xy[PL_GATHER], b_c[PL_GATHER];
    unsigned long long a_key[PL_GATHER], b_key[PL_GATHER];
    uint32_t s_ls[PL_CAP], s_le[PL_CAP], s_dirty[PL_CAP], s_clash[PL_CAP];
    int32_t s_tied[2 * TIE_CAP];
    unsigned long long s_pos[TIE_CAP];
    uint32_t s_lidx[TIE_CAP];
    uint32_t s_rows[PL_ROWS], s_cnt[8], s_r16[16], s_wtot[PL_CAP / 64];
    uint32_t s_fail, s_n, s_theta, s_nrows, s_nl, s_reach, s_k, s_unt, s_x;
    PoolScratch X;
    uint32_t s_sw[3 * CH_KMAX];
};
__device__ __forceinline__ void
pool_sel_body(uint32_t *__restrict__ rowmax, uint32_t *__restrict__ mat, uint32_t stride, DevState *st, const SlotRefH &ref,
              const CandArgs &C, uint32_t *__restrict__ dbits, unsigned long long *__restrict__ res, uint32_t tag,
              unsigned long long *__restrict__ req, uint32_t kcap, PoolEnt *__restrict__ pool, uint32_t *__restrict__ gather,
              uint32_t hint_below, long long *__restrict__ dpkey, unsigned long long dprank, PoolEnt *__restrict__ mid,
              PoolLds &L, const uint32_t blk, const uint32_t nblk, unsigned long long *dbg = nullptr, const bool aa_ok = false) {
    auto dstamp = [&](int i) {
        if (dbg && threadIdx.x == 0 && blk == 0) dbg[i] = wall_clock64();
    };
    auto &s_red = L.s_red;
    auto &s_words = L.s_words;
    auto &s_pref = L.s_pref;
    auto &s_exrow = L.s_exrow;
    auto &s_exm = L.s_exm;
    auto &s_exarg = L.s_exarg;
    auto &a_xy = L.a_xy;
    auto &a_c = L.a_c;
    auto &b_xy = L.b_xy;
    auto &b_c = L.b_c;
    auto &a_key = L.a_key;
    auto &b_key = L.b_key;
    auto &s_ls = L.s_ls;
    auto &s_le = L.s_le;
    auto &s_dirty = L.s_dirty;
    auto &s_clash = L.s_clash;
    auto &s_tied = L.s_tied;
    auto &s_pos = L.s_pos;
    auto &s_lidx = L.s_lidx;
    auto &s_rows = L.s_rows;
    auto &s_cnt = L.s_cnt;
    auto &s_r16 = L.s_r16;
    auto &s_wtot = L.s_wtot;
    uint32_t &s_fail = L.s_fail, &s_n = L.s_n, &s_theta = L.s_theta, &s_nrows = L.s_nrows, &s_nl = L.s_nl, &s_k = L.s_k, &s_reach = L.s_reach,
             &s_unt = L.s_unt, &s_x = L.s_x;
    const uint32_t tid = threadIdx.x;
    enum { PW_BB = CH_KMAX, PW_STATUS = 2 * CH_KMAX, PW_DEFER, PW_GAP, PW_ITER, PW_NM, PW_HINT, PW_THETA, PW_POOLN, PW_BK, PW_BZ0, PW_EPOCH_LO, PW_EPOCH_HI, PW_N };
    PoolEnt my_ent;
    my_ent.xy = my_ent.c = 0;
    my_ent.key = 0;
    if (blk == 0 && tid < PL_CAP) my_ent = pool[tid];
    if (tid < (uint32_t)PW_N) {
        const uint32_t *base = reinterpret_cast<const uint32_t *>(st);
        uint32_t off;
        if (tid < (uint32_t)PW_BB) off = (uint32_t)offsetof(DevState, ba) / 4 + tid;
        else if (tid < (uint32_t)PW_STATUS) off = (uint32_t)offsetof(DevState, bb) / 4 + (tid - (uint32_t)PW_BB);
        else {
            static_assert(PW_N <= 3 * CH_KMAX, "s_sw");
            constexpr uint32_t o[PW_N - PW_STATUS] = {
                (uint32_t)offsetof(DevState, status) / 4,     (uint32_t)offsetof(DevState, defer) / 4,      (uint32_t)offsetof(DevState, gap) / 4,
                (uint32_t)offsetof(DevState, iter) / 4,       (uint32_t)offsetof(DevState, num_merges) / 4, (uint32_t)offsetof(DevState, pool_hint) / 4,
                (uint32_t)offsetof(DevState, pool_theta) / 4, (uint32_t)offsetof(DevState, pool_n) / 4,     (uint32_t)offsetof(DevState, bk) / 4,
                (uint32_t)offsetof(DevState, bz0) / 4,        (uint32_t)offsetof(DevState, pool_epoch) / 4, (uint32_t)offsetof(DevState, pool_epoch) / 4 + 1};
            off = o[0];
#pragma unroll
            for (int k = 1; k < PW_N - PW_STATUS; k++) off = (tid == (uint32_t)PW_STATUS + (uint32_t)k) ? o[k] : off;
        }
        L.s_sw[tid] = base[off];
    }
    __syncthreads();
    const uint32_t *s_sw = L.s_sw;
    const uint32_t status = s_sw[PW_STATUS], defer = s_sw[PW_DEFER], gap = s_sw[PW_GAP];
    const uint32_t iter = s_sw[PW_ITER], nm = s_sw[PW_NM], hint = s_sw[PW_HINT];
    if (dpkey && blk == 0 && tid < (uint32_t)DP_KEY_WORDS)
        dpkey[tid] = tid == 0 ? -(long long)status : (tid == 1 ? 0ll : 0x7FFFFFFFFFFFFFFFll);
    if (status || defer) return;
    if (iter >= nm) {
        if (blk == 0 && tid == 0) st->bk = 0;
        return;
    }
    const uint32_t vcur = 256u + iter;
    const DirtyView D{s_words, s_pref};
    if (blk != 0) {
        if (!hint) return;
        const uint32_t nd = dirty_view_build(dbits, D);
        if (nd) lean_scan_rows(mat, stride, rowmax, vcur, NOROW, NOROW, NOROW, D, 3 + nd, blk - 1, nblk - 1, res, tag,
                               true, s_red, 3);
        if (tid == 0) {
            uint32_t n = 0, th = 0;
            if (!granule_get(req, tag, n)) n = 0;
            if (n && !granule_get(req + 1 + PL_ROWS, tag, th)) n = 0;
            s_n = n;
            s_theta = th;
        }
        __syncthreads();
        const uint32_t n = s_n, theta = s_theta;
        if (blk - 1 >= n) return;
        for (uint32_t j = blk - 1; j < n; j += nblk - 1) {
            if (tid == 0) {
                uint32_t x = 0;
                s_x = granule_get(req + 1 + j, tag, x) ? x : 0xFFFFFFFFu;
            }
            __syncthreads();
            const uint32_t x = s_x;
            if (x != 0xFFFFFFFFu) {
                const uint32_t *row = mat + (size_t)x * stride;
                const uint32_t n4 = (vcur + 3) & ~3u;
                constexpr int U = 8;
                for (uint32_t base = 0; base < n4; base += U * 4096) {
                    uint4 q[U];
#pragma unroll
                    for (int u = 0; u < U; u++) {
                        const uint32_t y = base + ((uint32_t)u * 1024u + tid) * 4u;
                        q[u] = (y < n4) ? *reinterpret_cast<const uint4 *>(row + y) : make_uint4(0u, 0u, 0u, 0u);
                    }
#pragma unroll
                    for (int u = 0; u < U; u++) {
                        const uint32_t y = base + ((uint32_t)u * 1024u + tid) * 4u;
                        const uint32_t v[4] = {q[u].x, q[u].y, q[u].z, q[u].w};
#pragma unroll
                        for (int k = 0; k < 4; k++) {
                            if (v[k] >= theta && y + k < vcur) {
                                const uint32_t s = atomicAdd(&gather[0], 1u);
                                if (s < PL_GATHER) {
                                    __hip_atomic_store(&gather[2 + 2 * s], (x << 16) | (y + k), __ATOMIC_RELAXED, __HIP_MEMORY_SCOPE_AGENT);
                                    __hip_atomic_store(&gather[3 + 2 * s], v[k], __ATOMIC_RELAXED, __HIP_MEMORY_SCOPE_AGENT);
                                }
                            }
                        }
                    }
                }
            }
            __syncthreads();
        }
        __builtin_amdgcn_s_waitcnt(0);
        __syncthreads();
        if (tid == 0) granule_put(req + 2 + PL_ROWS + blk, tag, 1u);
        return;
    }
    auto dismiss = [&]() {
        if (hint && tid == 0) granule_put(req, tag, 0u);
    };
    uint32_t rm[SEL_RPT];
    if (hint) select_load(rowmax, vcur, rm);
    uint32_t theta = s_sw[PW_THETA];
    unsigned long long epoch = (unsigned long long)s_sw[PW_EPOCH_LO] | ((unsigned long long)s_sw[PW_EPOCH_HI] << 32);
    const uint32_t n0 = min(s_sw[PW_POOLN], PL_CAP);
    if (tid == 0) {
        s_fail = 0;
        s_nrows = 0;
        s_nl = 0;
        s_unt = 0;
    }
    if (tid < 8) s_cnt[tid] = 0;
    dstamp(8);
    uint32_t vx[4] = {0, 0, 0, 0}, vy[4] = {0, 0, 0, 0}, cv[4] = {0, 0, 0, 0}, keepm = 0, ec = 0;
    unsigned long long ekey = 0;
    uint32_t mxm = 0, nmulti = 0;
    bool multi = false;
    auto multi_variants = [&](auto &&emit) {
        const uint32_t zp = s_sw[PW_BZ0];
        const uint32_t x = vx[0], y = vy[0];
        const bool hy = vy[2] != y;
        for (uint32_t m = mxm | 0x80000000u; m; m &= m - 1u) {
            const uint32_t p = (uint32_t)__ffs((int)m) - 1u;
            const uint32_t lx = p == 31u ? x : zp + p;
            for (uint32_t r = 0; r < (hy ? 2u : 1u); r++) {
                const uint32_t ry = r ? vy[2] : y;
                const uint32_t c = mat[(size_t)lx * stride + ry];
                if (c >= theta) emit(lx, ry, c);
            }
        }
    };
    if (tid < n0) {
        const uint32_t Kp = min(s_sw[PW_BK], (uint32_t)CH_KMAX), zp = s_sw[PW_BZ0];
        const PoolEnt e = my_ent;
        const uint32_t x = e.xy >> 16, y = e.xy & 0xFFFFu;
        ec = e.c;
        ekey = e.key;
        int32_t zx = -1, zy = -1;
        for (uint32_t p = 0; p < Kp; p++) {
            if (s_sw[PW_BB + p] == x) {
                zx = (int32_t)(zp + p);
                mxm |= 1u << p;
            }
            if (s_sw[p] == y) zy = (int32_t)(zp + p);
        }
        multi = (mxm & (mxm - 1u)) != 0;
        vx[0] = vx[2] = x;
        vx[1] = vx[3] = zx >= 0 ? (uint32_t)zx : x;
        vy[0] = vy[1] = y;
        vy[2] = vy[3] = zy >= 0 ? (uint32_t)zy : y;
        if (zx < 0 && zy < 0) {
            cv[0] = e.c;
            keepm = 1u;
        } else if (multi) {
            multi_variants([&](uint32_t, uint32_t, uint32_t) { nmulti++; });
        } else {
            const bool on[4] = {true, zx >= 0, zy >= 0, zx >= 0 && zy >= 0};
#pragma unroll
            for (int v = 0; v < 4; v++) cv[v] = on[v] ? mat[(size_t)vx[v] * stride + vy[v]] : 0u;
#pragma unroll
            for (int v = 0; v < 4; v++) keepm |= (on[v] && cv[v] >= theta) ? 1u << v : 0u;
        }
    }
    __syncthreads();
    {
        const uint32_t no = multi ? nmulti : (uint32_t)__popc(keepm);
        const uint32_t inc = wave_iscan_add(no);
        if (tid < PL_CAP && lane_id() == 63) s_wtot[wave_id()] = inc;
        __syncthreads();
        if (tid < PL_CAP) {
            uint32_t o = inc - no;
            for (int w = 0; w < wave_id(); w++) o += s_wtot[w];
            if (multi) {
                multi_variants([&](uint32_t lx, uint32_t ry, uint32_t c) {
                    if (o < PL_GATHER) {
                        a_xy[o] = (lx << 16) | ry;
                        a_c[o] = c;
                        a_key[o] = c == ec ? ekey : 0ull;
                    }
                    o++;
                });
            }
#pragma unroll
            for (int v = 0; v < 4; v++) {
                if ((keepm >> v) & 1u) {
                    if (o < PL_GATHER) {
                        a_xy[o] = (vx[v] << 16) | vy[v];
                        a_c[o] = cv[v];
                        a_key[o] = cv[v] == ec ? ekey : 0ull;
                    }
                    o++;
                }
            }
        }
        __syncthreads();
    }
    dstamp(9);
    uint32_t n1 = 0;
    if (n0) for (uint32_t w = 0; w < PL_CAP / 64; w++) n1 += s_wtot[w];
    if (n1 > PL_GATHER) n1 = 0;
    bool rebuilt = false;
    if (hint && n1 < min(kcap, nm - iter)) n1 = 0;
    if (n1 == 0) {
        if (!hint) {
            if (tid == 0) {
                st->bk = 0;
                st->found = 0;
                st->pool_n = 0;
                st->pool_hint_next = 1;
                st->sel_mode = CH_LIST;
                st->tl_n = st->tl_skip = 0;
            }
            return;
        }
        rebuilt = true;
        const uint32_t nd = dirty_view_build(dbits, D);
        if (tid == 0) st->sel_ran = 1;
        if (nd > CH_EX_CAP) {
            if (tid == 0) {
                st->found = 0;
                st->bk = 0;
                st->defer = 2;
            }
            dismiss();
            return;
        }
        for (uint32_t i = tid; i < nd; i += 1024) {
            const uint32_t x = dirty_view_row(D, i);
            uint32_t m = 0, arg = 0;
// ... 92 lines not shown
        __builtin_amdgcn_s_waitcnt(0);
        __syncthreads();
        const uint32_t nrows = min(s_nrows, PL_ROWS);
        if (tid < nrows) granule_put(req + 1 + tid, tag, s_rows[tid]);
        if (tid == 0) {
            granule_put(req + 1 + PL_ROWS, tag, theta);
            granule_put(req, tag, nrows);
        }
        const uint32_t nh = min(nblk - 1, nrows);
        if (tid < nh) {
            uint32_t d = 0;
            if (!granule_get(req + 2 + PL_ROWS + (tid + 1), tag, d)) s_fail = 1;
        }
        __syncthreads();
        if (s_fail) {
            if (tid == 0) atomicExch(&st->status, ST_LOOKBACK);
            return;
        }
        const uint32_t ng = __hip_atomic_load(&gather[0], __ATOMIC_RELAXED, __HIP_MEMORY_SCOPE_AGENT);
        if (ng > PL_GATHER || ng == 0) {
            if (tid == 0) {
                st->count = M;
                st->found = 0;
                st->bk = 0;
                if (ng) st->defer = 2; else atomicExch(&st->status, ST_INTERNAL);
            }
            return;
        }
        if (tid < ng) {
            a_xy[tid] = __hip_atomic_load(&gather[2 + 2 * tid], __ATOMIC_RELAXED, __HIP_MEMORY_SCOPE_AGENT);
            a_c[tid] = __hip_atomic_load(&gather[3 + 2 * tid], __ATOMIC_RELAXED, __HIP_MEMORY_SCOPE_AGENT);
            a_key[tid] = 0ull;
        }
        n1 = ng;
        __syncthreads();
    } else {
        dismiss();
        if (hint && tid == 0) st->sel_ran = 1;
    }
    dstamp(10);
    pool_sort(a_xy, a_c, a_key, b_xy, b_c, b_key, n1, L.X);
    dstamp(11);
    uint32_t n = n1;
    if (n1 > PL_CAP) {
        if (tid == 0) {
            uint32_t cut = PL_CAP;
            while (cut > 0 && b_c[cut - 1] == b_c[cut]) cut--;
            s_n = cut;
        }
        __syncthreads();
        n = s_n;
        if (n == 0) {
            if (tid == 0) {
                st->count = b_c[0];
                st->found = 0;
                st->bk = 0;
                st->defer = 2;
                st->pool_n = 0;
                st->pool_hint_next = 1;
            }
            return;
        }
        theta = b_c[n] + 1;
        __syncthreads();
    }
    const uint32_t kmax = min(kcap, nm - iter);
    const uint32_t nwalk = min(n, kmax);
    const int ksh = dpkey ? PL_KSH_DP : PL_KSH;
    PoolScratch &X = L.X;
    pool_level_bounds(b_c, n, s_ls, s_le, X);
    pool_levels_dirty(b_key, n, s_ls, s_le, s_dirty, ksh, X);
    if (tid < 64) s_clash[tid] = 0;
    if (tid == 0) {
        X.fv = 0xFFFFFFFFu;
        X.nl = 0;
    }
    __syncthreads();
    {
        const uint32_t t = tid & (PL_CAP - 1u);
        if (t < n) {
            const uint32_t x = b_xy[t] >> 16, y = b_xy[t] & 0xFFFFu;
            for (uint32_t i = tid / PL_CAP; i < nwalk; i += blockDim.x / PL_CAP) {
                const uint32_t xi = b_xy[i] >> 16, yi = b_xy[i] & 0xFFFFu;
                if (t != i && t < s_le[i] && ((xi == x) | (xi == y) | (yi == x))) s_clash[i] = 1;
            }
            if (tid < nwalk && x == y) s_clash[tid] = 1;
        }
    }
    __syncthreads();
    if (tid < 64) {
        const unsigned long long cb = __ballot(tid < nwalk && s_clash[tid] != 0);
        const uint32_t lim = cb ? (uint32_t)__ffsll((long long)cb) - 1u : nwalk - 1u;
        if (tid == 0) s_reach = s_le[lim];
    }
    __syncthreads();
    {
        const uint32_t reach = s_reach;
        const bool locate = dpkey || (C.T != 0 && gap == 0);
        const uint32_t scan_end = min(n, reach + 48u);
        const bool cons = locate && tid < n && s_ls[tid] < scan_end && s_dirty[tid] != 0;
        const uint32_t one = cons ? 1u : 0u;
        const uint32_t inc = wave_iscan_add(one);
        if (tid < PL_CAP && lane_id() == 63) X.wtot[wave_id()] = inc;
        __syncthreads();
        uint32_t P = inc - one;
        if (tid < PL_CAP)
            for (int v = 0; v < wave_id(); v++) P += X.wtot[v];
        if (cons && s_ls[tid] == tid) {
            const uint32_t size = s_le[tid] - tid;
            if ((tid >= reach && P + size > 16u) || P + size > (uint32_t)TIE_CAP) atomicMin(&X.fv, tid);
        }
        __syncthreads();
        const bool take = cons && s_ls[tid] < X.fv;
        if (take) {
            s_tied[2 * P] = (int32_t)(b_xy[tid] >> 16);
            s_tied[2 * P + 1] = (int32_t)(b_xy[tid] & 0xFFFFu);
            s_lidx[P] = tid;
        }
        if (tid < PL_CAP) {
            const unsigned long long tb = __ballot(take);
            if (lane_id() == 0 && tb) atomicAdd(&X.nl, (uint32_t)__popcll(tb));
        }
        __syncthreads();
        if (tid == 0) s_nl = X.nl;
        __syncthreads();
    }
    const uint32_t nl = s_nl;
    dstamp(12);
    if (dpkey) {
        const bool objection = nl != 0 && gap != 0;
        if (nl && !objection) (void)tie_by_index(ref, C, s_tied, nl, s_pos);
        __syncthreads();
        if (tid == 1 && objection) dpkey[1] = -1ll;
        if (tid < nl && !objection && s_pos[tid] != NOPOS)
            dpkey[2 + tid] = (long long)((dprank << PL_POS_DP) | (s_pos[tid] & ((1ull << PL_POS_DP) - 1ull)));
        if (tid < n) {
            PoolEnt e;
            e.xy = b_xy[tid];
            e.c = b_c[tid];
            e.key = b_key[tid];
            mid[1 + tid] = e;
        }
        if (tid < nl) mid[1 + PL_CAP + tid].xy = s_lidx[tid];
        if (tid == 0) {
            PoolEnt h;
            h.xy = n | (nl << 16);
            h.c = theta;
            h.key = epoch | ((unsigned long long)(rebuilt ? 1u : 0u) << 63);
            mid[0] = h;
            st->dp_wait = 1;
            st->bk = 0;
            st->found = 0;
        }
        return;
    }
    if (nl) {
        (void)tie_by_index(ref, C, s_tied, nl, s_pos);
        __syncthreads();
        epoch++;
        if (tid < nl) b_key[s_lidx[tid]] = s_pos[tid] != NOPOS ? (epoch << PL_KSH) | s_pos[tid] : 0ull;
        __syncthreads();
    }
    dstamp(13);
    pool_finish(st, pool, b_xy, b_c, b_key, a_xy, a_c, a_key, s_ls, s_le, s_dirty, s_clash, &s_k, &s_unt, n, kmax, iter, theta,
                epoch, rebuilt, hint_below, PL_KSH, X, aa_ok);
    dstamp(14);
}

__global__ void __launch_bounds__(1024)
k_pool_sel(uint32_t *__restrict__ rowmax, uint32_t *__restrict__ mat, uint32_t stride, DevState *st, SlotRefH ref,
           CandArgs C, uint32_t *__restrict__ dbits, unsigned long long *__restrict__ res, uint32_t tag,
           unsigned long long *__restrict__ req, uint32_t kcap, PoolEnt *__restrict__ pool, uint32_t *__restrict__ gather,
           uint32_t hint_below, long long *__restrict__ dpkey, unsigned long long dprank, PoolEnt *__restrict__ mid,
           uint32_t aa_ok) {
    __shared__ PoolLds L;
    pool_sel_body(rowmax, mat, stride, st, ref, C, dbits, res, tag, req, kcap, pool, gather, hint_below, dpkey, dprank, mid, L,
                  blockIdx.x, gridDim.x, nullptr, aa_ok != 0);
}

__global__ void __launch_bounds__(PL_CAP)
k_pool_sel_dp(DevState *st, const long long *__restrict__ key, uint32_t kcap, PoolEnt *__restrict__ pool,
              const PoolEnt *__restrict__ mid, uint32_t hint_below) {
    __shared__ uint32_t a_xy[PL_CAP], a_c[PL_CAP], b_xy[PL_CAP], b_c[PL_CAP];
    __shared__ unsigned long long a_key[PL_CAP], b_key[PL_CAP];
    __shared__ uint32_t s_ls[PL_CAP], s_le[PL_CAP], s_dirty[PL_CAP], s_clash[PL_CAP];
    __shared__ uint32_t s_k, s_unt;
    __shared__ PoolScratch X;
    const uint32_t tid = threadIdx.x;
    const uint32_t status = st->status;
    if (key[0] < 0 && status == 0) {
        if (tid == 0) st->status = ST_INTERNAL;
        return;
    }
    if (status || st->defer || !st->dp_wait) return;
    const PoolEnt h = mid[0];
    const uint32_t n = h.xy & 0xFFFFu, nl = h.xy >> 16, theta = h.c;
    unsigned long long epoch = h.key & 0x7FFFFFFFFFFFFFFFull;
    const bool rebuilt = (h.key >> 63) != 0;
    const uint32_t iter = st->iter, nm = st->num_merges;
    if (tid < n) {
        const PoolEnt e = mid[1 + tid];
        b_xy[tid] = e.xy;
        b_c[tid] = e.c;
        b_key[tid] = e.key;
    }
    __syncthreads();
    if (nl) {
        epoch++;
        const bool objection = key[1] < 0;
        if (tid < nl) {
            const long long p = key[2 + tid];
            b_key[mid[1 + PL_CAP + tid].xy] =
                (!objection && p != 0x7FFFFFFFFFFFFFFFll) ? (epoch << PL_KSH_DP) | (unsigned long long)p : 0ull;
        }
        __syncthreads();
    }
    pool_level_bounds(b_c, n, s_ls, s_le, X);
    pool_finish(st, pool, b_xy, b_c, b_key, a_xy, a_c, a_key, s_ls, s_le, s_dirty, s_clash, &s_k, &s_unt, n, min(kcap, nm - iter),
                iter, theta, epoch, rebuilt, hint_below, PL_KSH_DP, X);
}

}
}
```

### minbpe_amd/csrc/kernels/k_step.hip

```cpp
#include <hip/hip_runtime.h>
#include <stdint.h>

#include "../bpe_device.h"

namespace bpe {
namespace BPE_G {

constexpr uint32_t STEP_PUB_WORDS = 32;
constexpr int STEP_KCAP = 15;
static_assert(2 + 2 * STEP_KCAP == STEP_PUB_WORDS && STEP_KCAP <= CH_KSWEEP, "the line holds the pairs and their counts");

union StepLds {
    PoolLds p;
    MergeLds m;
};

__device__ __forceinline__ bool step_grid_barrier(uint32_t *ctr, uint32_t target, uint32_t *s_flag) {
    __builtin_amdgcn_s_waitcnt(0);
    __syncthreads();
    if (threadIdx.x == 0) {
        __hip_atomic_fetch_add(ctr, 1u, __ATOMIC_RELAXED, __HIP_MEMORY_SCOPE_AGENT);
        uint32_t ok = 0;
        for (uint32_t spins = 0; spins < LOOKBACK_SPINS; spins++) {
            if ((int32_t)(__hip_atomic_load(ctr, __ATOMIC_RELAXED, __HIP_MEMORY_SCOPE_AGENT) - target) >= 0) {
                ok = 1;
                break;
            }
            __builtin_amdgcn_s_sleep(1);
        }
        *s_flag = ok;
    }
    __syncthreads();
    return *s_flag != 0;
}

__global__ void __launch_bounds__(LEAN_MT)
k_step(StepArgs S) {
    __shared__ StepLds U;
    __shared__ uint32_t s_b[STEP_PUB_WORDS], s_adj[CH_KMAX];
    __shared__ uint32_t s_flag;
    DevState *st = S.st;
    const uint32_t tid = threadIdx.x;
    const int swho = blockIdx.x == 0 ? 0 : (blockIdx.x == S.gm / 2 ? 1 : (blockIdx.x == gridDim.x - 1 ? 2 : -1));
    auto stamp = [&](int i) {
        if (S.stamps && tid == 0 && swho >= 0) S.stamps[(((size_t)(S.step % STEP_STAMP_RING)) * 3 + (size_t)swho) * 16 + (size_t)i] = wall_clock64();
    };
    unsigned long long *const dbg = (S.stamps && swho >= 0) ? S.stamps + (((size_t)(S.step % STEP_STAMP_RING)) * 3 + (size_t)swho) * 16 : nullptr;
    stamp(0);
    if (blockIdx.x == 0) {
        pool_sel_body(S.rowmax, S.mat, S.stride, st, S.ref, S.C, S.dbits, S.res, S.tag, S.req, S.kcap, S.pool, S.gather,
                      S.hint_below, nullptr, 0ull, S.pool + PL_CAP, U.p, 0u, 1u + S.nscan, dbg);
        __builtin_amdgcn_s_waitcnt(0);
        __syncthreads();
        stamp(1);
        if (tid < STEP_PUB_WORDS) {
            const uint32_t status = st->status, defer = st->defer;
            const uint32_t noop = (status || defer) ? 1u : 0u;
            const uint32_t K = noop ? 0u : min(st->bk, (uint32_t)STEP_KCAP);
            uint32_t v = 0;
            if (tid == 0)
                v = K | (st->brep << 8) | ((st->sel_ran ? 1u : 0u) << 16) | (noop << 17) | ((st->pool_hint_next ? 1u : 0u) << 18) |
                    ((defer & 3u) << 19) | ((st->sel_mode & 1u) << 21);
            else if (tid == 1) v = 256u + st->iter;
            else if (tid - 2 < K) v = ((uint32_t)st->ba[tid - 2] << 16) | ((uint32_t)st->bb[tid - 2] & 0xFFFFu);
            else if (tid >= 2 + STEP_KCAP && tid - (2 + STEP_KCAP) < K) v = st->bcnt[tid - (2 + STEP_KCAP)];
            s_b[tid] = v;
            granule_put(S.pub + tid, S.tag, v);
        }
        if (tid == 0) s_flag = 1;
    } else {
        if (blockIdx.x <= S.nscan)
            pool_sel_body(S.rowmax, S.mat, S.stride, st, S.ref, S.C, S.dbits, S.res, S.tag, S.req, S.kcap, S.pool, S.gather,
                          S.hint_below, nullptr, 0ull, S.pool + PL_CAP, U.p, blockIdx.x, 1u + S.nscan);
        __syncthreads();
        if (tid == 0) s_flag = 1;
        __syncthreads();
        if (tid < STEP_PUB_WORDS) {
            uint32_t v = 0;
            if (!granule_get(S.pub + tid, S.tag, v)) s_flag = 0;
            s_b[tid] = v;
        }
    }
    __syncthreads();
    if (!s_flag) {
        if (tid == 0) atomicExch(&st->status, ST_LOOKBACK);
        if (tid < STEP_PUB_WORDS) s_b[tid] = tid == 0 ? (1u << 17) : 0u;
    }
    __syncthreads();
    stamp(2);
    if (S.stamps && tid == 0 && blockIdx.x < 256)
        S.stamps[(size_t)STEP_STAMP_RING * 3 * 16 + ((size_t)(S.step % STEP_STAMP_RING) * 256 + blockIdx.x) * 2] = wall_clock64();
    const uint32_t K = s_b[0] & 0xFFu, brep = (s_b[0] >> 8) & 0xFFu, ran = (s_b[0] >> 16) & 1u, z0 = s_b[1];
    const bool sel_noop = ((s_b[0] >> 17) & 1u) != 0 || K == 0;
    if (!sel_noop && blockIdx.x < S.gm) {
        MergeLds &L = U.m;
        if (tid < CH_KMAX) {
            const uint32_t w = tid < K ? s_b[2 + tid] : 0u;
            L.s_pa[tid] = tid < K ? (w >> 16) : 0xFFFFFFFFu;
            L.s_pb[tid] = tid < K ? (w & 0xFFFFu) : 0xFFFFFFFFu;
            L.s_pb1[tid + 1] = tid < K ? (w & 0xFFFFu) : 0xFFFFFFFFu;
            if (tid == 0) L.s_pb1[0] = 0xFFFFFFFFu;
        }
        __syncthreads();
        merge_chain_body<true>(S.A, S.idx_dirty, S.use_index, L, K, z0, brep, blockIdx.x, S.gm, blockIdx.x == 0 ? nullptr : dbg);
    }
    stamp(3);
    if (S.stamps && tid == 0 && blockIdx.x < 256) {
        unsigned long long *all = S.stamps + (size_t)STEP_STAMP_RING * 3 * 16 + ((size_t)(S.step % STEP_STAMP_RING) * 256 + blockIdx.x) * 2;
        all[1] = wall_clock64();
    }
    const bool arrived = step_grid_barrier(S.bar, S.bar_target, &s_flag);
    stamp(4);
    if (!arrived && tid == 0) atomicExch(&st->status, ST_LOOKBACK);
    const uint32_t status = arrived ? ld_agent(&st->status) : (uint32_t)ST_LOOKBACK;
    const bool noop = status || ((s_b[0] >> 19) & 3u) || K == 0;
    if (!noop) {
        const uint32_t nwv4 = (((z0 + K - 1u) >> 8) + 1u) * 4u;
        const uint32_t wpw = (nwv4 + gridDim.x - 1u) / gridDim.x;
        const uint32_t tw = blockIdx.x * wpw + (uint32_t)wave_id();
        if (tid < CH_KMAX) s_adj[tid] = K == 1 ? (tid == 0 ? ld_agent(&st->adj) : 0u) : (tid < K ? ld_agent(&st->badj[tid]) : 0u);
        __syncthreads();
        if ((uint32_t)wave_id() < wpw && tw < nwv4)
            apply_chain_tokens<true>(tw * 64u + (uint32_t)lane_id(), S.mat, S.stride, S.delta, S.dl, S.rowmax, S.dbits, S.sums,
                                     nullptr, 0u, nullptr, K, z0, ran, s_b + 2, s_adj, brep);
    } else if (ran && arrived) {
        for (uint32_t i = blockIdx.x * (uint32_t)LEAN_MT + tid; i < (uint32_t)DBITS_WORDS; i += gridDim.x * (uint32_t)LEAN_MT) S.dbits[i] = 0;
    }
    stamp(5);
    if ((blockIdx.x == 0 || blockIdx.x == gridDim.x - 1) && wave_id() == 0) {
        const uint32_t lane = (uint32_t)lane_id();
        const uint32_t defer2 = (s_b[0] >> 19) & 3u, mode_used = (s_b[0] >> 21) & 1u, hint_next = (s_b[0] >> 18) & 1u;
        uint32_t v = 0;
        if (S.removed) {
#pragma unroll
            for (int i = 0; i < 4; i++) v += ld_agent(&S.removed[(lane * 4 + i) * REMOVED_STRIDE]);
        }
        static_assert(CH_RMV == 8, "lanes 2p, 2p + 1 hold the removals of pair p");
        const uint32_t tot = wave_sum_u32(v);
        v += (uint32_t)__shfl_xor((int)v, 1);
        uint32_t rem[STEP_KCAP + 1];
#pragma unroll
        for (int p = 0; p < STEP_KCAP + 1; p++) rem[p] = (uint32_t)__shfl((int)v, 2 * p);
        if (K == 1) rem[0] = tot;
        if (!S.removed) {
#pragma unroll
            for (int p = 0; p < STEP_KCAP + 1; p++) rem[p] = p < STEP_KCAP ? s_b[2 + STEP_KCAP + p] : 0u;
        }
        const uint32_t iter = z0 - 256u;
        unsigned long long nn = st->n[S.par];
        if (!noop)
            for (uint32_t p = 0; p < K; p++) nn -= rem[p];
        if (blockIdx.x == 0) {
            if (S.removed && lane < 64) {
#pragma unroll
                for (int i = 0; i < 4; i++) S.removed[(lane * 4 + i) * REMOVED_STRIDE] = 0;
            }
            if (lane == 0) {
                if (!noop) st->iter = iter + K;
                if (status == 0) st->n[S.par ^ 1] = nn;
                st->removed = 0;
                st->pool_hint = hint_next;
                if (arrived) st->sel_ran = 0;
            }
        }
        if (blockIdx.x == gridDim.x - 1 && lane == 0) {
            if (!noop) {
                unsigned long long m = st->n[S.par];
                for (uint32_t p = 0; p < K; p++) {
                    m -= rem[p];
                    iter_rec_put(S.rec + iter + p, (int32_t)(s_b[2 + p] >> 16), (int32_t)(s_b[2 + p] & 0xFFFFu), s_b[2 + STEP_KCAP + p], ST_OK, m);
                }
                __builtin_amdgcn_s_waitcnt(0);
                for (uint32_t p = 0; p < K; p++) iter_rec_seal(S.rec + iter + p, (unsigned long long)(iter + p) + 1);
                __builtin_amdgcn_s_waitcnt(0);
            }
            StepRec *sr = S.srec + (S.step % STEP_RING);
            step_rec_put(sr, iter, noop ? 0u : K, (status == 0 && defer2) ? (uint32_t)ST_DEFER : status, mode_used | (defer2 << 8), nn);
            __builtin_amdgcn_s_waitcnt(0);
            step_rec_seal(sr, (unsigned long long)S.step + 1);
        }
    }
    stamp(6);
    if (noop) return;
    apply_chain_commit<true>(blockIdx.x * (uint32_t)LEAN_MT + tid, gridDim.x * (uint32_t)LEAN_MT, S.nwords, S.smask, S.stage, S.hdr_cur);
// ... 6 lines not shown
```

Before: 57480 merges/s.

## Allow chained merges sharing a first token via pair-keyed hash lookup

Relaxes the chain-independence check so several merges in one chained step may share the same left token, letting more merges be batched per step. To support this, the per-step merge lookup is rekeyed on the (a,b) pair rather than on a alone, using a two-word hash entry. The hash table is also used for smaller K (default minimum 2 instead of 5), and the multi-variant candidate enumeration now covers repeated right tokens. This adds per-token hash work and a larger shared-memory table, and risks correctness issues where overlapping merges interact.

```diff
diff --git a/minbpe_amd/_native.py b/minbpe_amd/_native.py
--- a/minbpe_amd/_native.py
+++ b/minbpe_amd/_native.py
@@ -493,11 +493,12 @@
         self._check(_lib.bpe_prof_reset(self._h))
 
     def train_stats(self):
-        out = np.zeros(12, np.uint64)
-        self._check(_lib.bpe_train_stats_ex(self._h, _ptr(out), 12))
+        out = np.zeros(13, np.uint64)
+        self._check(_lib.bpe_train_stats_ex(self._h, _ptr(out), 13))
         return dict(dense=int(out[0]), sparse=int(out[1]), index_builds=int(out[2]), slots=int(out[3]),
                     lean=int(out[4]), deferred=int(out[5]), chained=int(out[6]), steps=int(out[7]),
-                    selections=int(out[8]), slot_ids=int(out[9]), fused_steps=int(out[10]), aa_in_chain=int(out[11]))
+                    selections=int(out[8]), slot_ids=int(out[9]), fused_steps=int(out[10]), aa_in_chain=int(out[11]),
+                    shared_first=int(out[12]))
 
     def prof_read(self):
         k = len(PROF_KINDS)
diff --git a/minbpe_amd/csrc/api/api_basic.hip b/minbpe_amd/csrc/api/api_basic.hip
--- a/minbpe_amd/csrc/api/api_basic.hip
+++ b/minbpe_amd/csrc/api/api_basic.hip
@@ -196,6 +196,12 @@
     } else if (!strcmp(name, "chain_aa")) {
         if (value < 0 || value > 1) return fail(c, BPE_E_ARG, "chain_aa must be 0 or 1");
         c->chain_aa = (int)value;
+    } else if (!strcmp(name, "chain_share_first")) {
+        if (value < 0 || value > 1) return fail(c, BPE_E_ARG, "chain_share_first must be 0 or 1");
+        c->chain_share_first = (int)value;
+    } else if (!strcmp(name, "chain_hash_kmin")) {
+        if (value < 0 || value > 32) return fail(c, BPE_E_ARG, "chain_hash_kmin must be 0..32");
+        c->chain_hash_kmin = (int)value;
     } else if (!strcmp(name, "pool_hint")) {
         if (value < 0 || value > 128) return fail(c, BPE_E_ARG, "pool_hint must be 0..128");
         c->pool_hint = (int)value;
diff --git a/minbpe_amd/csrc/api/api_ctx.hip b/minbpe_amd/csrc/api/api_ctx.hip
--- a/minbpe_amd/csrc/api/api_ctx.hip
+++ b/minbpe_amd/csrc/api/api_ctx.hip
@@ -123,6 +123,9 @@
     uint64_t n_fused = 0;
     int chain_aa = 1;
     uint64_t n_aa_chain = 0;
+    int chain_share_first = 1;
+    int chain_hash_kmin = 0;
+    uint64_t n_shared_first = 0;
     unsigned long long *d_step_stamps = nullptr;
     int pool_hint = 0;
     PoolEnt *d_pool = nullptr;
@@ -1101,6 +1104,8 @@
     const unsigned nscan = (unsigned)std::max(1, std::min(c->chain_scan, c->num_cus - 1));
     const bool aa_on = c->chain_aa && !fused && !c->forced && !dense && !dp && c->lean == 1 && c->idx_live && c->aa_sparse &&
                        c->ts == TILE2_MIN && c->d_desc != nullptr;
+    const bool share_first = c->chain_share_first && !fused && !c->forced && !dp;
+    const uint32_t sel_flags = (aa_on ? (uint32_t)PSF_AA : 0u) | (share_first ? (uint32_t)PSF_SHARE_FIRST : 0u) | ((uint32_t)c->chain_hash_kmin << 8);
     if (fused) {
         if (!c->d_step_pub) {
             HIPCHK(c, hipMalloc((void **)&c->d_step_pub, 64 * sizeof(unsigned long long)));
@@ -1191,7 +1196,7 @@
         hipLaunchKernelGGL(GK(c, k_pool_sel), dim3(1 + nscan), dim3(1024), 0, c->stream, c->d_rowmax, c->d_mat,
                            c->vcap, c->d_st, stream_ref_h(c), C, c->d_dbits, c->d_lean_res, ++c->lean_tag, c->d_chain_req,
                            kcap, c->d_pool, c->d_pool_gather, hint_below, dp ? c->d_dp_ckey : (long long *)nullptr,
-                           (unsigned long long)(dp ? dp->rank : 0), c->d_pool + PL_CAP, aa_on ? 1u : 0u);
+                           (unsigned long long)(dp ? dp->rank : 0), c->d_pool + PL_CAP, sel_flags);
     LAUNCHCHK(c, "k_pool_sel");
     if (dp) {
         TRY(dp_allreduce(c, c->d_dp_ckey, DP_KEY_WORDS, BPE_DT_INT64, BPE_OP_MIN));
diff --git a/minbpe_amd/csrc/api/api_prof.hip b/minbpe_amd/csrc/api/api_prof.hip
--- a/minbpe_amd/csrc/api/api_prof.hip
+++ b/minbpe_amd/csrc/api/api_prof.hip
@@ -40,9 +40,10 @@
         TRY(read_state(c, &stt));
         chained = stt.chain_taken;
     }
-    const uint64_t v[12] = {c->n_dense, c->n_sparse, c->n_index_builds, c->slot_T, c->n_lean, c->n_deferred,
-                            chained + c->n_chained, c->n_steps, c->n_full, (uint64_t)c->ts, c->n_fused, c->n_aa_chain};
-    for (int i = 0; i < n && i < 12; i++) out[i] = v[i];
+    const uint64_t v[13] = {c->n_dense, c->n_sparse, c->n_index_builds, c->slot_T, c->n_lean, c->n_deferred,
+                            chained + c->n_chained, c->n_steps, c->n_full, (uint64_t)c->ts, c->n_fused, c->n_aa_chain,
+                            c->n_shared_first};
+    for (int i = 0; i < n && i < 13; i++) out[i] = v[i];
     return BPE_OK;
 }
 
diff --git a/minbpe_amd/csrc/api/api_rccl.hip b/minbpe_amd/csrc/api/api_rccl.hip
--- a/minbpe_amd/csrc/api/api_rccl.hip
+++ b/minbpe_amd/csrc/api/api_rccl.hip
@@ -121,6 +121,7 @@
     uint64_t lean_at_last_defer = 0, n_chain_merges = 0;
     c->n_lean = c->n_deferred = 0;
     c->n_aa_chain = 0;
+    c->n_shared_first = 0;
     c->n_steps = c->n_full = c->n_chained = 0;
     c->rows_pending = false;
     c->sum_valid = false;
diff --git a/minbpe_amd/csrc/api/api_train.hip b/minbpe_amd/csrc/api/api_train.hip
--- a/minbpe_amd/csrc/api/api_train.hip
+++ b/minbpe_amd/csrc/api/api_train.hip
@@ -59,6 +59,7 @@
     c->n_steps = c->n_full = c->n_chained = 0;
     c->n_fused = 0;
     c->n_aa_chain = 0;
+    c->n_shared_first = 0;
     static const char *stamp_path = getenv("BPE_STEP_STAMPS");
     const size_t stamp_bytes = (size_t)STEP_STAMP_RING * (3 * 16 + 256 * 2) * sizeof(unsigned long long);
     if (stamp_path) {
@@ -324,6 +325,12 @@
                         TRY(take_record((int)(sr.first_iter + j), true));
                         if (!stop && c->h_rec[sr.first_iter + j].a == c->h_rec[sr.first_iter + j].b) c->n_aa_chain++;
                     }
+                    if (sr.k > 1 && !stop) {
+                        bool twice = false;
+                        for (uint32_t j = 1; j < sr.k && !twice; j++)
+                            for (uint32_t i = 0; i < j && !twice; i++) twice = c->h_rec[sr.first_iter + i].a == c->h_rec[sr.first_iter + j].a;
+                        if (twice) c->n_shared_first++;
+                    }
                     if (sr.k) {
                         c->n_lean += sr.k;
                         if ((sr.pad & 0xFF) == CH_FULL) c->n_full++;
diff --git a/minbpe_amd/csrc/kernels/k_chain.hip b/minbpe_amd/csrc/kernels/k_chain.hip
--- a/minbpe_amd/csrc/kernels/k_chain.hip
+++ b/minbpe_amd/csrc/kernels/k_chain.hip
@@ -16,6 +16,12 @@
     return (w0 == INVALID_WORD) ? -1 : hit;
 }
 
+__device__ __forceinline__ uint32_t chain_hash_m2(uint32_t m) { return 2u * m * m + 1u; }
+__device__ __forceinline__ uint32_t chain_pair_bucket(uint32_t a, uint32_t b, uint32_t m, uint32_t m2) {
+    return ((__umul24(a, m) + __umul24(b, m2)) >> 8) & 255u;
+}
+constexpr uint32_t CH_HASH_KMIN = 2;
+
 constexpr uint32_t CH_DCAP = 1024;
 constexpr uint32_t CH_SD = 2 * CH_DCAP + 2;
 __device__ __forceinline__ void chain_slot_load(const AbArgs &A, const uint32_t t, uint4 (&rv)[MJ], uint4 &hv) {
@@ -29,10 +35,10 @@
 }
 template <bool DENSE, bool THROUGH = false>
 __device__ __forceinline__ void merge_chain_wave(uint32_t *__restrict__ out, uint32_t *__restrict__ sd, const uint32_t t, const AbArgs &A,
-                                                 const uint32_t *pa, const uint32_t *pb, const uint32_t *pb1,
+                                                 const uint32_t *pa, const uint32_t *pb,
                                                  const uint32_t K, const uint32_t z0, const uint32_t brep,
                                                  uint4 (&rv)[MJ], const uint4 hv,
-                                                 const uint32_t *ph = nullptr, const uint32_t hm = 0,
+                                                 const uint2 *ph = nullptr, const uint32_t hm = 0,
                                                  const uint32_t tl_in = 0xFFFFFFFFu) {
     const int lane = lane_id();
     const uint32_t Tl = tl_in != 0xFFFFFFFFu ? tl_in : min(A.T, A.st->tlive);
@@ -100,47 +106,46 @@
         jc[j] = 0;
     }
     uint32_t s = 0;
-    uint32_t ia[MJ];
-#pragma unroll
-    for (int j = 0; j < MJ; j++) ia[j] = 0;
     uint32_t ip = 0;
+    uint32_t nxw[MJ];
+#pragma unroll
+    for (int j = 0; j < MJ; j++) {
+        const uint32_t up = (j < MJ - 1) ? lane_first(x[(j + 1) % MJ][0]) : tail[0];
+        nxw[j] = lane_next(x[j][0], up);
+    }
     if (hm) {
-        auto code = [&](uint32_t w) -> uint32_t {
+        const uint32_t hm2 = chain_hash_m2(hm);
+        auto code = [&](uint32_t w, uint32_t nx) -> uint32_t {
             const uint32_t id = w & IDMASK;
-            const uint32_t e = ph[(__umul24(id, hm) >> 8) & 255u];
-            return (e >> 8) == id ? (e & 255u) : 0u;
+            const uint2 e = ph[chain_pair_bucket(id, nx & IDMASK, hm, hm2)];
+            return ((e.x >> 8) == id && e.y == (nx & NWMASK)) ? (e.x & 255u) : 0u;
         };
 #pragma unroll
         for (int j = 0; j < MJ; j++) {
 #pragma unroll
-            for (int k = 0; k < 4; k++) ia[j] |= code(x[j][k]) << (8 * k);
-        }
-        ip = code(prev1);
+            for (int k = 0; k < 4; k++) jc[j] |= code(x[j][k], (k < 3) ? x[j][(k + 1) & 3] : nxw[j]) << (8 * k);
+        }
+        ip = code(prev1, first);
     } else {
         for (uint32_t p = 0; p < K; p++) {
-            const uint32_t a = pa[p];
+            const uint32_t a = pa[p], b = pb[p];
 #pragma unroll
             for (int j = 0; j < MJ; j++) {
 #pragma unroll
-                for (int k = 0; k < 4; k++) ia[j] |= ((x[j][k] & IDMASK) == a) ? (p + 1u) << (8 * k) : 0u;
-            }
-            ip = ((prev1 & IDMASK) == a) ? p + 1u : ip;
+                for (int k = 0; k < 4; k++) {
+                    const uint32_t nxt = (k < 3) ? x[j][(k + 1) & 3] : nxw[j];
+                    jc[j] |= (((x[j][k] & IDMASK) == a) & ((nxt & NWMASK) == b)) ? (p + 1u) << (8 * k) : 0u;
+                }
+            }
+            ip = (((prev1 & IDMASK) == a) & ((first & NWMASK) == b)) ? p + 1u : ip;
         }
     }
 #pragma unroll
     for (int j = 0; j < MJ; j++) {
-        const uint32_t up = (j < MJ - 1) ? lane_first(x[(j + 1) % MJ][0]) : tail[0];
-        const uint32_t nxw = lane_next(x[j][0], up);
-#pragma unroll
-        for (int k = 0; k < 4; k++) {
-            const uint32_t nxt = (k < 3) ? x[j][k + 1] : nxw;
-            const uint32_t i = (ia[j] >> (8 * k)) & 255u;
-            const uint32_t m = (uint32_t)((nxt & NWMASK) == pb1[i]);
-            rb[j] |= m << k;
-            jc[j] |= (m ? i : 0u) << (8 * k);
-        }
-    }
-    s = (uint32_t)((prev1 != INVALID_WORD) & ((first & NWMASK) == pb1[ip]));
+#pragma unroll
+        for (int k = 0; k < 4; k++) rb[j] |= (uint32_t)(((jc[j] >> (8 * k)) & 255u) != 0u) << k;
+    }
+    s = (uint32_t)((prev1 != INVALID_WORD) & (ip != 0u));
 #pragma unroll
     for (int j = 0; j < MJ; j++) {
         const int nb = (int)len - (j * 256 + lane * 4);
@@ -460,14 +465,16 @@
     __builtin_amdgcn_wave_barrier();
 }
 
-__device__ __forceinline__ uint32_t chain_hash_find(const uint32_t *pa, uint32_t K, uint32_t *tab) {
-    if (K < 5) return 0u;
+__device__ __forceinline__ uint32_t chain_hash_find(const uint32_t *pa, const uint32_t *pb, uint32_t K, uint32_t *tab,
+                                                    uint32_t kmin = CH_HASH_KMIN) {
+    if (K < kmin) return 0u;
     const uint32_t lane = (uint32_t)lane_id(), half = lane >> 5, l = lane & 31u;
     const bool in = l < K;
-    const uint32_t a = in ? pa[l] : 0u;
+    const uint32_t a = in ? pa[l] : 0u, b = in ? pb[l] : 0u;
     volatile uint32_t *t = tab + half * 256u;
     for (uint32_t m = 129u; m < 256u; m += 4u) {
-        const uint32_t h = (__umul24(a, m + 2u * half) >> 8) & 255u;
+        const uint32_t mm = m + 2u * half;
+        const uint32_t h = chain_pair_bucket(a, b, mm, chain_hash_m2(mm));
         if (in) t[h] = l;
         __builtin_amdgcn_fence(__ATOMIC_RELEASE, "wavefront");
         __builtin_amdgcn_wave_barrier();
@@ -479,15 +486,15 @@
     }
     return 0u;
 }
-__device__ __forceinline__ uint32_t chain_hash_build(uint32_t *s_ph, uint32_t *s_hm, uint32_t *s_hs, const uint32_t *s_pa, uint32_t K,
-                                                     bool pre_ok = false, uint32_t pre_hm = 0) {
-    if (threadIdx.x < 256) s_ph[threadIdx.x] = 0xFFFFFFFFu;
+__device__ __forceinline__ uint32_t chain_hash_build(uint2 *s_ph, uint32_t *s_hm, uint32_t *s_hs, const uint32_t *s_pa,
+                                                     const uint32_t *s_pb, uint32_t K, bool pre_ok = false, uint32_t pre_hm = 0) {
+    if (threadIdx.x < 256) s_ph[threadIdx.x] = make_uint2(0xFFFFFFFFu, 0xFFFFFFFFu);
     uint32_t hm = pre_hm;
     if (!pre_ok) {
         if (threadIdx.x == 0) *s_hm = 0;
         __syncthreads();
         if (wave_id() == 0) {
-            const uint32_t f = chain_hash_find(s_pa, K, s_hs);
+            const uint32_t f = chain_hash_find(s_pa, s_pb, K, s_hs);
             if (lane_id() == 0) *s_hm = f;
         }
         __syncthreads();
@@ -495,7 +502,9 @@
     } else {
         __syncthreads();
     }
-    if (hm && threadIdx.x < K) s_ph[(__umul24(s_pa[threadIdx.x], hm) >> 8) & 255u] = (s_pa[threadIdx.x] << 8) | (threadIdx.x + 1u);
+    if (hm && threadIdx.x < K)
+        s_ph[chain_pair_bucket(s_pa[threadIdx.x], s_pb[threadIdx.x], hm, chain_hash_m2(hm))] =
+            make_uint2((s_pa[threadIdx.x] << 8) | (threadIdx.x + 1u), s_pb[threadIdx.x]);
     __syncthreads();
     return hm;
 }
@@ -504,8 +513,9 @@
     alignas(16) uint32_t s_out[LEAN_MT / 64][TILE2];
     uint32_t s_list[LEAN_SUB * 32];
     uint32_t s_tot[2];
-    uint32_t s_pa[CH_KMAX], s_pb[CH_KMAX], s_pb1[CH_KMAX + 1];
-    uint32_t s_ph[256], s_hm;
+    uint32_t s_pa[CH_KMAX], s_pb[CH_KMAX];
+    alignas(8) uint2 s_ph[256];
+    uint32_t s_hm;
     uint32_t s_hs[512];
 };
 template <bool THROUGH = false>
@@ -523,9 +533,8 @@
     auto &s_tot = L.s_tot;
     auto &s_pa = L.s_pa;
     auto &s_pb = L.s_pb;
-    auto &s_pb1 = L.s_pb1;
-    const uint32_t hm = chain_hash_build(L.s_ph, &L.s_hm, L.s_hs, s_pa, K, pre_ok, pre_hm);
-    const uint32_t *s_ph = L.s_ph;
+    const uint32_t hm = chain_hash_build(L.s_ph, &L.s_hm, L.s_hs, s_pa, s_pb, K, pre_ok, pre_hm);
+    const uint2 *s_ph = L.s_ph;
     const uint32_t Tl = min(A.T, have_st ? tlive_in : st->tlive);
     const uint32_t gap = have_st ? gap_in : st->gap;
     constexpr uint32_t NWV = LEAN_MT / 64;
@@ -545,7 +554,7 @@
         } else {
             uint4 rv[MJ], hv;
             chain_slot_load(A, t, rv, hv);
-            merge_chain_wave<false, THROUGH>(s_out[wave_id()], nullptr, t, A, s_pa, s_pb, s_pb1, K, z0, brep, rv, hv, s_ph, hm, Tl);
+            merge_chain_wave<false, THROUGH>(s_out[wave_id()], nullptr, t, A, s_pa, s_pb, K, z0, brep, rv, hv, s_ph, hm, Tl);
         }
     };
     if (!(use_index & 1u) || gap != 0) {
@@ -604,7 +613,7 @@
             for (; i < n; i += NWV) {
                 const bool more = i + NWV < n;
                 if (more) chain_slot_load(A, s_list[i + NWV], nrv, nhv);
-                merge_chain_wave<false, THROUGH>(s_out[wave_id()], nullptr, s_list[i], A, s_pa, s_pb, s_pb1, K, z0, brep, rv, hv, s_ph, hm, Tl);
+                merge_chain_wave<false, THROUGH>(s_out[wave_id()], nullptr, s_list[i], A, s_pa, s_pb, K, z0, brep, rv, hv, s_ph, hm, Tl);
                 if (more) {
 #pragma unroll
                     for (int j = 0; j < MJ; j++) rv[j] = nrv[j];
@@ -658,8 +667,6 @@
     if (threadIdx.x < CH_KMAX) {
         L.s_pa[threadIdx.x] = threadIdx.x < K ? s_w[threadIdx.x] : 0xFFFFFFFFu;
         L.s_pb[threadIdx.x] = threadIdx.x < K ? s_w[SW_BB + threadIdx.x] : 0xFFFFFFFFu;
-        L.s_pb1[threadIdx.x + 1] = threadIdx.x < K ? s_w[SW_BB + threadIdx.x] : 0xFFFFFFFFu;
-        if (threadIdx.x == 0) L.s_pb1[0] = 0xFFFFFFFFu;
     }
     __syncthreads();
     if (K == 1 && s_w[0] == s_w[SW_BB] && !(MJ == 1 && X.on)) {
@@ -676,7 +683,7 @@
 k_merge_chain_dense(AbArgs A, uint32_t *__restrict__ dbits) {
     __shared__ __attribute__((aligned(16))) uint32_t s_out[LEAN_MT / 64][TILE2];
     __shared__ uint32_t s_sd[CH_KDENSE * CH_SD];
-    __shared__ uint32_t s_pa[CH_KMAX], s_pb[CH_KMAX], s_pb1[CH_KMAX + 1];
+    __shared__ uint32_t s_pa[CH_KMAX], s_pb[CH_KMAX];
     DevState *st = A.st;
     const uint32_t ran = st->sel_ran;
     if (blockIdx.x == 0 && ran) {
@@ -697,8 +704,6 @@
     if (threadIdx.x < CH_KMAX) {
         s_pa[threadIdx.x] = threadIdx.x < K ? (uint32_t)st->ba[threadIdx.x] : 0xFFFFFFFFu;
         s_pb[threadIdx.x] = threadIdx.x < K ? (uint32_t)st->bb[threadIdx.x] : 0xFFFFFFFFu;
-        s_pb1[threadIdx.x + 1] = threadIdx.x < K ? (uint32_t)st->bb[threadIdx.x] : 0xFFFFFFFFu;
-        if (threadIdx.x == 0) s_pb1[0] = 0xFFFFFFFFu;
     }
     for (uint32_t i = threadIdx.x; i < K * CH_SD; i += LEAN_MT) s_sd[i] = 0;
     __syncthreads();
@@ -709,7 +714,7 @@
     {
         uint4 rv[MJ], hv;
         chain_slot_load(A, t, rv, hv);
-        merge_chain_wave<true>(s_out[wave_id()], s_sd, t, A, s_pa, s_pb, s_pb1, K, z0, (uint32_t)CH_RSTRIDE, rv, hv, nullptr, 0, Tl);
+        merge_chain_wave<true>(s_out[wave_id()], s_sd, t, A, s_pa, s_pb, K, z0, (uint32_t)CH_RSTRIDE, rv, hv, nullptr, 0, Tl);
     }
     __syncthreads();
     const uint32_t vc = A.vcap & 0xFFFFFFu;
@@ -1127,10 +1132,13 @@
     const uint32_t K = bb ? min(kcap, (uint32_t)__ffsll((long long)bb) - 1u) : kcap;
     const uint32_t c = lane < K ? mat[(size_t)a * stride + b] : 0u;
     const uint32_t cmax = wave_umax_dpp(c);
-    __shared__ uint32_t s_pa[CH_KMAX], s_hs[512];
-    if (lane < CH_KMAX) s_pa[lane] = a;
+    __shared__ uint32_t s_pa[CH_KMAX], s_pb[CH_KMAX], s_hs[512];
+    if (lane < CH_KMAX) {
+        s_pa[lane] = a;
+        s_pb[lane] = b;
+    }
     __syncthreads();
-    const uint32_t hm = chain_hash_find(s_pa, K, s_hs);
+    const uint32_t hm = chain_hash_find(s_pa, s_pb, K, s_hs);
     if (lane == 0) {
         st_agent(&st->adj, 0u);
         st->count = c;
diff --git a/minbpe_amd/csrc/kernels/k_pool.hip b/minbpe_amd/csrc/kernels/k_pool.hip
--- a/minbpe_amd/csrc/kernels/k_pool.hip
+++ b/minbpe_amd/csrc/kernels/k_pool.hip
@@ -104,7 +104,8 @@
                                             unsigned long long *a_key, const uint32_t *s_ls, const uint32_t *s_le,
                                             uint32_t *s_dirty, uint32_t *s_clash, uint32_t *s_k, uint32_t *s_unt, uint32_t n,
                                             uint32_t kmax, uint32_t iter, uint32_t theta, unsigned long long epoch, bool rebuilt,
-                                            uint32_t hint_below, int ksh, PoolScratch &X, const bool aa_ok = false) {
+                                            uint32_t hint_below, int ksh, PoolScratch &X, const bool aa_ok = false,
+                                            const bool share_first = false, const uint32_t hash_kmin = CH_HASH_KMIN) {
     const uint32_t tid = threadIdx.x;
     const uint32_t nwalk = min(n, kmax);
     const uint32_t sh = blockDim.x >= 4 * PL_CAP ? 2u : 0u;
@@ -152,7 +153,7 @@
         } else if (j < i) {
             const uint32_t xj = a_xy[j] >> 16, yj = a_xy[j] & 0xFFFFu;
             if (j == 0 && xj == yj) bad = true;
-            bad |= (xj == x) | (xj == y) | (yj == x);
+            bad |= ((xj == x) & !share_first) | (xj == y) | (yj == x);
         }
         if (bad) atomicOr(&X.bad, 1u << i);
     }
@@ -185,7 +186,10 @@
         }
     }
     if (K == 0) return;
-    if (tid < K) X.rank[tid] = a_xy[tid] >> 16;
+    if (tid < K) {
+        X.rank[tid] = a_xy[tid] >> 16;
+        X.rank[CH_KMAX + tid] = a_xy[tid] & 0xFFFFu;
+    }
     __syncthreads();
     if (tid < 64) {
         uint32_t c = 0;
@@ -197,7 +201,7 @@
             st->bcnt[tid] = c;
         }
         const uint32_t cmax = wave_umax_dpp(c);
-        const uint32_t hm = chain_hash_find(reinterpret_cast<const uint32_t *>(X.rank), K, X.rank + 256);
+        const uint32_t hm = chain_hash_find(X.rank, X.rank + CH_KMAX, K, X.rank + 256, hash_kmin);
         if (tid == 0) {
             st->brep = cmax > CH_REP_COUNT ? (uint32_t)CH_RSTRIDE : (uint32_t)CH_REP;
             st->bhm = hm;
@@ -231,6 +235,7 @@
     }
 }
 
+enum : uint32_t { PSF_AA = 1u, PSF_SHARE_FIRST = 2u };
 struct PoolLds {
     unsigned long long s_red[32];
     uint32_t s_words[DBITS_WORDS], s_pref[DBITS_WORDS + 1];
@@ -251,7 +256,9 @@
               const CandArgs &C, uint32_t *__restrict__ dbits, unsigned long long *__restrict__ res, uint32_t tag,
               unsigned long long *__restrict__ req, uint32_t kcap, PoolEnt *__restrict__ pool, uint32_t *__restrict__ gather,
               uint32_t hint_below, long long *__restrict__ dpkey, unsigned long long dprank, PoolEnt *__restrict__ mid,
-              PoolLds &L, const uint32_t blk, const uint32_t nblk, unsigned long long *dbg = nullptr, const bool aa_ok = false) {
+              PoolLds &L, const uint32_t blk, const uint32_t nblk, unsigned long long *dbg = nullptr, const uint32_t flags = 0) {
+    const bool aa_ok = (flags & PSF_AA) != 0, share_first = (flags & PSF_SHARE_FIRST) != 0;
+    const uint32_t hash_kmin = (flags >> 8) ? (flags >> 8) : CH_HASH_KMIN;
     auto dstamp = [&](int i) {
         if (dbg && threadIdx.x == 0 && blk == 0) dbg[i] = wall_clock64();
     };
@@ -392,17 +399,17 @@
     dstamp(8);
     uint32_t vx[4] = {0, 0, 0, 0}, vy[4] = {0, 0, 0, 0}, cv[4] = {0, 0, 0, 0}, keepm = 0, ec = 0;
     unsigned long long ekey = 0;
-    uint32_t mxm = 0, nmulti = 0;
+    uint32_t mxm = 0, mym = 0, nmulti = 0;
     bool multi = false;
     auto multi_variants = [&](auto &&emit) {
         const uint32_t zp = s_sw[PW_BZ0];
         const uint32_t x = vx[0], y = vy[0];
-        const bool hy = vy[2] != y;
         for (uint32_t m = mxm | 0x80000000u; m; m &= m - 1u) {
             const uint32_t p = (uint32_t)__ffs((int)m) - 1u;
             const uint32_t lx = p == 31u ? x : zp + p;
-            for (uint32_t r = 0; r < (hy ? 2u : 1u); r++) {
-                const uint32_t ry = r ? vy[2] : y;
+            for (uint32_t m2 = mym | 0x80000000u; m2; m2 &= m2 - 1u) {
+                const uint32_t q = (uint32_t)__ffs((int)m2) - 1u;
+                const uint32_t ry = q == 31u ? y : zp + q;
                 const uint32_t c = mat[(size_t)lx * stride + ry];
                 if (c >= theta) emit(lx, ry, c);
             }
@@ -420,9 +427,12 @@
                 zx = (int32_t)(zp + p);
                 mxm |= 1u << p;
             }
-            if (s_sw[p] == y) zy = (int32_t)(zp + p);
-        }
-        multi = (mxm & (mxm - 1u)) != 0;
+            if (s_sw[p] == y) {
+                zy = (int32_t)(zp + p);
+                mym |= 1u << p;
+            }
+        }
+        multi = ((mxm & (mxm - 1u)) | (mym & (mym - 1u))) != 0;
         vx[0] = vx[2] = x;
         vx[1] = vx[3] = zx >= 0 ? (uint32_t)zx : x;
         vy[0] = vy[1] = y;
@@ -681,7 +691,7 @@
             const uint32_t x = b_xy[t] >> 16, y = b_xy[t] & 0xFFFFu;
             for (uint32_t i = tid / PL_CAP; i < nwalk; i += blockDim.x / PL_CAP) {
                 const uint32_t xi = b_xy[i] >> 16, yi = b_xy[i] & 0xFFFFu;
-                if (t != i && t < s_le[i] && ((xi == x) | (xi == y) | (yi == x))) s_clash[i] = 1;
+                if (t != i && t < s_le[i] && (((xi == x) & !share_first) | (xi == y) | (yi == x))) s_clash[i] = 1;
             }
             if (tid < nwalk && x == y) s_clash[tid] = 1;
         }
@@ -762,7 +772,7 @@
     }
     dstamp(13);
     pool_finish(st, pool, b_xy, b_c, b_key, a_xy, a_c, a_key, s_ls, s_le, s_dirty, s_clash, &s_k, &s_unt, n, kmax, iter, theta,
-                epoch, rebuilt, hint_below, PL_KSH, X, aa_ok);
+                epoch, rebuilt, hint_below, PL_KSH, X, aa_ok, share_first, hash_kmin);
     dstamp(14);
 }
 
@@ -771,10 +781,10 @@
            CandArgs C, uint32_t *__restrict__ dbits, unsigned long long *__restrict__ res, uint32_t tag,
            unsigned long long *__restrict__ req, uint32_t kcap, PoolEnt *__restrict__ pool, uint32_t *__restrict__ gather,
            uint32_t hint_below, long long *__restrict__ dpkey, unsigned long long dprank, PoolEnt *__restrict__ mid,
-           uint32_t aa_ok) {
+           uint32_t flags) {
     __shared__ PoolLds L;
     pool_sel_body(rowmax, mat, stride, st, ref, C, dbits, res, tag, req, kcap, pool, gather, hint_below, dpkey, dprank, mid, L,
-                  blockIdx.x, gridDim.x, nullptr, aa_ok != 0);
+                  blockIdx.x, gridDim.x, nullptr, flags);
 }
 
 __global__ void __launch_bounds__(PL_CAP)
diff --git a/minbpe_amd/csrc/kernels/k_step.hip b/minbpe_amd/csrc/kernels/k_step.hip
--- a/minbpe_amd/csrc/kernels/k_step.hip
+++ b/minbpe_amd/csrc/kernels/k_step.hip
@@ -98,8 +98,6 @@
             const uint32_t w = tid < K ? s_b[2 + tid] : 0u;
             L.s_pa[tid] = tid < K ? (w >> 16) : 0xFFFFFFFFu;
             L.s_pb[tid] = tid < K ? (w & 0xFFFFu) : 0xFFFFFFFFu;
-            L.s_pb1[tid + 1] = tid < K ? (w & 0xFFFFu) : 0xFFFFFFFFu;
-            if (tid == 0) L.s_pb1[0] = 0xFFFFFFFFu;
         }
         __syncthreads();
         merge_chain_body<true>(S.A, S.idx_dirty, S.use_index, L, K, z0, brep, blockIdx.x, S.gm, blockIdx.x == 0 ? nullptr : dbg);
```

Result: faster. 60740 merges/s, median of 6 (+5.7%).
